# LanceZPF/loongx

Measured on AMD Instinct MI355X. Metric: edited images/s @512x512, 28-step Flux denoise, higher is better.
Workload: dtype bf16

## Files before the change

### include/lx.h

```cpp
#ifndef LX_H_
#define LX_H_
#include <stddef.h>
#include <stdint.h>
#ifdef __cplusplus
extern "C" {
#endif

#define LX_VERSION 404

typedef enum lx_status {
  LX_OK = 0,
  LX_ERR_INVALID = -1,
  LX_ERR_UNSUPPORTED = -2,
  LX_ERR_LAUNCH = -3,
  LX_ERR_NO_DEVICE = -4
} lx_status;

int lx_version(void);
const char* lx_last_error(void);
int lx_device_arch(char* name, size_t n);

enum {
  LX_EPI_STORE_BF16 = 0,
  LX_EPI_STORE_F32 = 1,
  LX_EPI_RESID_F32 = 2,
  LX_EPI_GELU = 0x100,
  LX_W_TILED = 0x200,
  LX_EPI_SPLIT_BF16 = 0x400,
  LX_EPI_STORE_FP8 = 3,
  LX_EPI_QKV = 0x1000,
  LX_OPERANDS_FP8 = 0x800,
  LX_OPERANDS_F16 = 0x2000
};

typedef struct lx_gemm_desc {
  const void* A;
  const void* W;
  const float* bias;
  void* C;
  const float* gate;
  const float* lora_t;
  const float* lora_up;
  int32_t M, N, K;
  int32_t lda, ldw, ldc;
  int32_t rows_per_batch, gate_ld;
  int32_t lora_r, lora_ldt, lora_mod_cols, lora_toff_max;
  int32_t epilogue;
  int32_t gelu_col_start;
  int32_t lora_nsplit;
  int32_t lora_split_stride;
  int32_t k_segs, a_lo_off;
  int32_t c_lo_off;
  float out_scale;
  union {
    const float* col_scale;
    int32_t* f16_ovf;
  };
  const float* qkv_norm_q;
  const float* qkv_norm_k;
  const float* qkv_rope;
  void* qkv_vt;
  void* qkv_k;
  int32_t qkv_d, qkv_vt_ld, qkv_vt_pos0;
  int32_t qkv_k_ld;
  void* qkv_q8;
  void* qkv_k8;
  void* qkv_vt8;
  int32_t qkv_ld8;
  float qkv_q_scale, qkv_k_scale, qkv_v_scale;
} lx_gemm_desc;

#define LX_GEMM_MAX_GROUP 4
int lx_gemm_bf16(const lx_gemm_desc* problems, int n, void* stream);
void lx_gemm_reload_env(void);

size_t lx_gemm_workspace_bytes(void);
int lx_gemm_bf16_ws(const lx_gemm_desc* problems, int n, void* workspace, size_t ws_bytes, void* stream);
int lx_gemm_workspace_status(void* workspace, void* stream);
enum { LX_GEMM_PLAN_NONE = 0, LX_GEMM_PLAN_8WAVE_256 = 1, LX_GEMM_PLAN_8WAVE_128 = 2, LX_GEMM_PLAN_MIXED = 3, LX_GEMM_PLAN_MIXED_2L = 4,
       LX_GEMM_PLAN_G4 = 5, LX_GEMM_PLAN_G4_SPLIT2 = 6, LX_GEMM_PLAN_G4_SPLIT3 = 7 };
int lx_gemm_last_plan(void);

int lx_lora_down(const void* X, int ldx, const void* Adown, float* T, int ldt, int M, int K, int R, int n_split,
                 int split_stride, void* stream);
int lx_lora_down_f16(const void* X, int ldx, const void* Adown, float* T, int ldt, int M, int K, int R, int n_split,
                     int split_stride, void* stream);
int lx_lora_down_terms(const void* const* X, const int* ldx, const void* const* Adown, int n_terms, float* T, int ldt, int M, int K, int R,
                       int slab_stride, void* stream);
typedef struct lx_rowscale_seg { int32_t row0, n_rows, rows_per_batch, _pad; } lx_rowscale_seg;
int lx_lora_scale_rows(float* T, int ldt, int R, int n_slab, int slab_stride, const lx_rowscale_seg* seg, int n_seg,
                       const float* W, int w_ld, int n_batches, int period, void* stream);

int lx_linear_skinny(const float* X, int ldx, const void* W, int ldw, const float* bias, float* Y, int ldy,
                     int M, int N, int K, int act_in, int act_out, int accumulate, void* stream);

int lx_timestep_embed(const float* t, float* out, int B, int dim, void* stream);

int lx_rope_table(const float* ids, int L, int a0, int a1, int a2, double theta, float* cos_t, float* sin_t, void* stream);

int lx_ln_modulate(const float* X, int ldx, const float* shift, const float* scale, int mod_ld, void* Y, int ldy,
                   int M, int D, int rows_per_batch, float eps, void* stream);
typedef struct lx_ln_seg { int32_t row0, n_rows, rows_per_batch, _pad; const float* shift; const float* scale; } lx_ln_seg;
int lx_ln_modulate_segs(const float* X, int ldx, const lx_ln_seg* seg, int n_seg, int mod_ld, void* Y, int ldy, int D,
                        float eps, void* stream);
int lx_ln_modulate_f16_segs(const float* X, int ldx, const lx_ln_seg* seg, int n_seg, int mod_ld, void* Y, int ldy, int D,
                            float eps, int32_t* f16_ovf, void* stream);
int lx_ln_modulate_lora_segs(const float* X, int ldx, const lx_ln_seg* seg, int n_seg, int mod_ld, void* Y, int ldy, int D,
                             float eps, const void* Adown, int R, float* T, int ldt, int lora_row0, int lora_rows, void* stream);
int lx_ln_modulate_lora_f16_segs(const float* X, int ldx, const lx_ln_seg* seg, int n_seg, int mod_ld, void* Y, int ldy, int D,
                                 float eps, const void* Adown, int R, float* T, int ldt, int lora_row0, int lora_rows,
                                 int32_t* f16_ovf, void* stream);
int lx_ln_modulate_delta(const float* X, int ldx, const float* shift, const float* scale, int mod_ld, float* P, int ldp,
                         int M, int D, int rows_per_batch, float eps, float* row_sums , double* sums , void* stream);

int lx_qkv_prep(void* QKV, int ld, int q_col, int k_col, int v_col, int row0, int n_rows, int rows_per_batch,
                int H, const float* wq, const float* wk, float eps, const float* cos_tab, const float* sin_tab,
                void* VT, int vt_ld, int vt_pos0, void* stream);

typedef struct lx_qkv_seg {
  int32_t row0, rows_per_batch, vt_pos0, _pad;
  const float* wq; const float* wk; const float* cos_tab; const float* sin_tab;
} lx_qkv_seg;
int lx_qkv_prep_segs(void* QKV, int ld, int q_col, int k_col, int v_col, const lx_qkv_seg* seg, int n_seg, int n_batches,
                     int H, float eps, void* VT, int vt_ld, void* stream);
int lx_qkv_prep_f16in_segs(void* QKV, int ld, int q_col, int k_col, int v_col, const lx_qkv_seg* seg, int n_seg, int n_batches,
                           int H, float eps, void* VT, int vt_ld, void* stream);

int lx_qkv_prep_kv_segs(void* QKV, int ld, int q_col, int k_col, int v_col, const lx_qkv_seg* seg, int n_seg, int n_batches,
                        int H, float eps, void* K2, int ldk2, int k2_col, void* VT, int vt_ld, void* stream);
int lx_qkv_prep_kv_f16in_segs(void* QKV, int ld, int q_col, int k_col, int v_col, const lx_qkv_seg* seg, int n_seg, int n_batches,
                              int H, float eps, void* K2, int ldk2, int k2_col, void* VT, int vt_ld, void* stream);

typedef struct lx_attn_desc {
  const void* Q; const void* K; const void* VT; void* O;
  int32_t ldq, ldk, ldo, vt_ld;
  int32_t q_col, k_col, o_col;
  int32_t B, H;
  int32_t n_seg;
  int32_t seg_row0[3], seg_len[3], seg_vt0[3];
  float bias[3][3];
  float scale;
  int32_t n_qseg;
  int32_t flags;
  int32_t qseg_mask;
  int32_t* f16_ovf;
} lx_attn_desc;
enum { LX_ATTN_Q_LOG2 = 1, LX_ATTN_BOUNDED = 2, LX_ATTN_INVARIANT = 4, LX_ATTN_O_F16 = 8, LX_ATTN_PREFER_4WAVE = 16, LX_ATTN_P_EXP2 = 32 };
int lx_attn_fwd(const lx_attn_desc* d, void* stream);
enum { LX_ATTN_KERNEL_NONE = 0, LX_ATTN_KERNEL_8WAVE = 1, LX_ATTN_KERNEL_4WAVE = 2 };
int lx_attn_last_kernel(void);

enum { LX_ATTN_MASK_BOOL = 0, LX_ATTN_MASK_F32 = 1, LX_ATTN_MASK_BF16 = 2, LX_ATTN_MASK_F16 = 3 };
typedef struct lx_attn_mask_desc {
  const void* mask;
  int32_t dtype;
  int32_t dims[4];
  int32_t _pad;
  int64_t strides[4];
  void* workspace;
  size_t workspace_bytes;
} lx_attn_mask_desc;
int lx_attn_mask_workspace(const lx_attn_desc* d, const lx_attn_mask_desc* m, size_t* bytes);
int lx_attn_mask_prep(const lx_attn_desc* d, const lx_attn_mask_desc* m, void* stream);
int lx_attn_fwd_masked(const lx_attn_desc* d, const lx_attn_mask_desc* m, void* stream);

int lx_qkv_prep_fp8_segs(const void* QKV, int ld, int q_col, int k_col, int v_col, const lx_qkv_seg* seg, int n_seg,
                         int n_batches, int H, float eps, void* Q8, void* K8, int ld8, void* VT8, int vt8_ld,
                         float q_scale, float k_scale, float v_scale, void* stream);
int lx_qkv_prep_fp8_f16in_segs(const void* QKV, int ld, int q_col, int k_col, int v_col, const lx_qkv_seg* seg, int n_seg,
                               int n_batches, int H, float eps, void* Q8, void* K8, int ld8, void* VT8, int vt8_ld,
                               float q_scale, float k_scale, float v_scale, void* stream);
int lx_attn_fwd_fp8(const lx_attn_desc* d, float qk_descale, float v_descale, void* stream);

int lx_split_bf16(const float* src, int lds, void* dst, int ldd, int lo_off, int M, int K, void* stream);
int lx_ln_modulate_split_segs(const float* X, int ldx, const lx_ln_seg* seg, int n_seg, int mod_ld, void* Y, int ldy, int y_lo_off,
                              int D, float eps, void* stream);
int lx_qkv_prep_f32_segs(float* QKV, int ld, int q_col, int k_col, const lx_qkv_seg* seg, int n_seg, int n_batches, int H, float eps,
                         void* stream);
typedef struct lx_attn_f32_desc {
  const float* QKV; int32_t ld, q_col, k_col, v_col;
  void* O; int32_t ldo, o_col, o_lo_off;
  int32_t B, H, n_seg;
  int32_t seg_row0[3], seg_len[3];
  float bias[3][3];
  float scale;
} lx_attn_f32_desc;
int lx_attn_fwd_f32(const lx_attn_f32_desc* d, void* stream);

int lx_qkv_prep_split_segs(const float* QKV, int ld, int q_col, int k_col, int v_col, const lx_qkv_seg* seg, int n_seg, int n_batches, int H,
                           float eps, void* QK2, int ld2, int q2_col, int k2_col, int lo_off, void* VT2, int vt_ld, long long vt_lo_off,
                           void* stream);
int lx_qkv_prep_split_kv_segs(const float* QKV, int ld, int q_col, int k_col, int v_col, const lx_qkv_seg* seg, int n_seg, int n_batches, int H,
                              float eps, void* Q2, int ldq2, int q2_col, void* K2, int ldk2, int k2_col, int lo_off, void* VT2, int vt_ld,
                              long long vt_lo_off, void* stream);
int lx_attn_fwd_split(const lx_attn_desc* d, int qk_lo_off, long long vt_lo_off, int o_lo_off, void* stream);

int lx_ln_modulate_fp8_segs(const float* X, int ldx, const lx_ln_seg* seg, int n_seg, int mod_ld, void* Y, int ldy, void* Y8, int ldy8,
                            float y8_scale, int D, float eps, void* stream);
int lx_convert_fp8(const void* src, int src_is_bf16, int lds, void* dst, int ldd, float scale, int M, int K, void* stream);
int lx_lora_down_fp8(const void* X8, int ldx, float x_descale, const void* Adown, float* T, int ldt, int M, int K, int R, int n_split,
                     int split_stride, void* stream);

int lx_euler_step(float* x, const void* v, int v_is_bf16, float dsigma, size_t n, void* stream);
int lx_scale_noise(float* out, const float* x0, const float* z, float sigma, size_t n, void* stream);
int lx_euler_step_blend(float* x, const void* v, int v_is_bf16, float dsigma, const float* x0, const float* z, const float* m,
                        float sigma_next, size_t n, void* stream);
int lx_euler_step_cfg(float* x, const void* v, int v_is_bf16, float dsigma, float scale, const float* x0, const float* z, const float* m,
                      float sigma_next, size_t n, void* stream);
int lx_euler_step_cfg3(float* x, const void* v, int v_is_bf16, float dsigma, float scale_brain, float scale_text, const float* x0,
                       const float* z, const float* m, float sigma_next, size_t n, void* stream);
int lx_euler_step_apg(float* x, const void* v, int v_is_bf16, int n_parts, float scale_a, float scale_b, float sigma, float dsigma, float eta,
                      float norm_threshold, float momentum, float* M, double* sums, void* workspace, size_t workspace_bytes, const float* x0,
                      const float* z, const float* m, float sigma_next, int n_images, size_t elems, void* stream);
size_t lx_apg_workspace_bytes(int n_images, size_t elems);
int lx_convert(void* dst, int dst_bf16, const void* src, int src_bf16, size_t n, void* stream);

int lx_s4_scan(const float* u, const double* lam, const double* w, const float* Dskip, float* y,
               int B, int H, int L, int N, void* stream);
int lx_s4_conv(const float* u, const float* Kker, const float* Dskip, float* y, int B, int H, int L, void* stream);
int lx_chanmix(const float* x, const float* W, const float* bias, const float* resid, const float* ln_g,
               const float* ln_b, float* y, int B, int Hin, int Hout, int L, int act, void* stream);
int lx_pyramid_pool(const float* x, float* y, int B, int C, int L, const int* sizes, int n_sizes, int ldy, int y_col0,
                    void* stream);
int lx_layernorm_relu(float* x, const float* g, const float* b, int M, int D, float eps, void* stream);
int lx_linear_f32(const float* X, int ldx, int x_trans, const float* W, int ldw, const float* bias, float* Y, int ldy,
                  int y_trans, int M, int N, int K, int accumulate, void* stream);

int lx_chan_gemm_f32(const float* X, long x_bstride, int ldx, const float* W, int ldw, const float* bias, float* Y, long y_bstride,
                     int ldy, int B, int N, int K, int L, int epilogue, float* part, void* stream);

size_t lx_duan_workspace_bytes(int B, int C, int L, int Hd);
int lx_duan_fwd(const float* x, const float* c, const float* gw1, const float* gb1, const float* gw2, const float* gb2,
                const float* mw1, const float* mb1, const float* mw2, const float* mb2, float* y,
                int B, int C, int L, int Hd, float eps, int keep_k, void* ws, size_t ws_bytes, void* stream);

size_t lx_groupnorm_workspace_bytes(int B, int P, int G);
int lx_groupnorm_silu(const void* x, int x_is_bf16, int B, int P, int C, int G, const float* gamma, const float* beta, float eps,
                      int silu, void* y, void* ws, size_t ws_bytes, void* stream);
int lx_im2col3x3(const void* x, int B, int H, int W, int C, int mode, void* out, int Kpad, void* stream);
int lx_softmax_rows(const float* S, int lds, float scale, void* P, int ldp, int M, int N, void* stream);
int lx_softmax_rows_valid(const float* S, int lds, float scale, void* P, int ldp, int M, int n_valid, int n_store, void* stream);

int lx_groupnorm_silu_split(const float* x, int B, int P, int C, int G, const float* gamma, const float* beta, float eps, int silu,
                            void* y, int ldy, int y_lo_off, void* ws, size_t ws_bytes, void* stream);
int lx_im2col3x3_split(const void* x, int ldx, int x_lo_off, int B, int H, int W, int C, int mode, void* out, int Kpad, void* stream);
int lx_softmax_rows_split(const float* S, int lds, float scale, void* P, int ldp, int p_lo_off, int M, int n_valid, int n_store, void* stream);

int lx_groupnorm_silu_f16(const float* x, int B, int P, int C, int G, const float* gamma, const float* beta, float eps, int silu, void* y,
                          void* ws, size_t ws_bytes, int32_t* f16_ovf, void* stream);
int lx_softmax_rows_f16(const float* S, int lds, float scale, void* P, int ldp, int M, int n_valid, int n_store, void* stream);
int lx_convert_f16(void* dst, const void* src, int src_bf16, size_t n, int32_t* f16_ovf, void* stream);

#ifdef __cplusplus
}
#endif
#endif
```

### loongx_amd/_lib.py

```python
from __future__ import annotations

import ctypes as C
import os

import torch

_HERE = os.path.dirname(os.path.abspath(__file__))
LIB_PATH = os.environ.get("LX_AMD_LIB", os.path.join(_HERE, "lib", "liblx_amd.so"))

LX_EPI_STORE_BF16, LX_EPI_STORE_F32, LX_EPI_RESID_F32, LX_EPI_GELU, LX_W_TILED, LX_EPI_SPLIT_BF16 = 0, 1, 2, 0x100, 0x200, 0x400
LX_EPI_STORE_FP8, LX_OPERANDS_FP8, LX_EPI_QKV, LX_OPERANDS_F16 = 3, 0x800, 0x1000, 0x2000
LX_GEMM_MAX_GROUP = 4
(LX_GEMM_PLAN_NONE, LX_GEMM_PLAN_8WAVE_256, LX_GEMM_PLAN_8WAVE_128, LX_GEMM_PLAN_MIXED, LX_GEMM_PLAN_MIXED_2L, LX_GEMM_PLAN_G4,
 LX_GEMM_PLAN_G4_SPLIT2, LX_GEMM_PLAN_G4_SPLIT3) = range(8)


class GemmDesc(C.Structure):
    _fields_ = [("A", C.c_void_p), ("W", C.c_void_p), ("bias", C.c_void_p), ("C", C.c_void_p),
                ("gate", C.c_void_p), ("lora_t", C.c_void_p), ("lora_up", C.c_void_p),
                ("M", C.c_int32), ("N", C.c_int32), ("K", C.c_int32),
                ("lda", C.c_int32), ("ldw", C.c_int32), ("ldc", C.c_int32),
                ("rows_per_batch", C.c_int32), ("gate_ld", C.c_int32),
                ("lora_r", C.c_int32), ("lora_ldt", C.c_int32), ("lora_mod_cols", C.c_int32),
                ("lora_toff_max", C.c_int32), ("epilogue", C.c_int32), ("gelu_col_start", C.c_int32),
                ("lora_nsplit", C.c_int32), ("lora_split_stride", C.c_int32),
                ("k_segs", C.c_int32), ("a_lo_off", C.c_int32), ("c_lo_off", C.c_int32), ("out_scale", C.c_float),
                ("col_scale", C.c_void_p),
                ("qkv_norm_q", C.c_void_p), ("qkv_norm_k", C.c_void_p), ("qkv_rope", C.c_void_p), ("qkv_vt", C.c_void_p),
                ("qkv_k", C.c_void_p),
                ("qkv_d", C.c_int32), ("qkv_vt_ld", C.c_int32), ("qkv_vt_pos0", C.c_int32), ("qkv_k_ld", C.c_int32),
                ("qkv_q8", C.c_void_p), ("qkv_k8", C.c_void_p), ("qkv_vt8", C.c_void_p),
                ("qkv_ld8", C.c_int32), ("qkv_q_scale", C.c_float), ("qkv_k_scale", C.c_float), ("qkv_v_scale", C.c_float)]


class AttnDesc(C.Structure):
    _fields_ = [("Q", C.c_void_p), ("K", C.c_void_p), ("VT", C.c_void_p), ("O", C.c_void_p),
                ("ldq", C.c_int32), ("ldk", C.c_int32), ("ldo", C.c_int32), ("vt_ld", C.c_int32),
                ("q_col", C.c_int32), ("k_col", C.c_int32), ("o_col", C.c_int32),
                ("B", C.c_int32), ("H", C.c_int32), ("n_seg", C.c_int32),
                ("seg_row0", C.c_int32 * 3), ("seg_len", C.c_int32 * 3), ("seg_vt0", C.c_int32 * 3),
                ("bias", (C.c_float * 3) * 3), ("scale", C.c_float), ("n_qseg", C.c_int32), ("flags", C.c_int32),
                ("qseg_mask", C.c_int32), ("f16_ovf", C.c_void_p)]


LX_ATTN_Q_LOG2, LX_ATTN_BOUNDED, LX_ATTN_INVARIANT, LX_ATTN_O_F16, LX_ATTN_PREFER_4WAVE, LX_ATTN_P_EXP2 = 1, 2, 4, 8, 16, 32
LX_ATTN_MASK_BOOL, LX_ATTN_MASK_F32, LX_ATTN_MASK_BF16, LX_ATTN_MASK_F16 = 0, 1, 2, 3


class AttnMaskDesc(C.Structure):
    _fields_ = [("mask", C.c_void_p), ("dtype", C.c_int32), ("dims", C.c_int32 * 4), ("_pad", C.c_int32),
                ("strides", C.c_int64 * 4), ("workspace", C.c_void_p), ("workspace_bytes", C.c_size_t)]


class AttnF32Desc(C.Structure):
    _fields_ = [("QKV", C.c_void_p), ("ld", C.c_int32), ("q_col", C.c_int32), ("k_col", C.c_int32), ("v_col", C.c_int32),
                ("O", C.c_void_p), ("ldo", C.c_int32), ("o_col", C.c_int32), ("o_lo_off", C.c_int32),
                ("B", C.c_int32), ("H", C.c_int32), ("n_seg", C.c_int32),
                ("seg_row0", C.c_int32 * 3), ("seg_len", C.c_int32 * 3),
                ("bias", (C.c_float * 3) * 3), ("scale", C.c_float)]


class LnSeg(C.Structure):
    _fields_ = [("row0", C.c_int32), ("n_rows", C.c_int32), ("rows_per_batch", C.c_int32), ("_pad", C.c_int32),
                ("shift", C.c_void_p), ("scale", C.c_void_p)]


class RowScaleSeg(C.Structure):
    _fields_ = [("row0", C.c_int32), ("n_rows", C.c_int32), ("rows_per_batch", C.c_int32), ("_pad", C.c_int32)]


class QkvSeg(C.Structure):
    _fields_ = [("row0", C.c_int32), ("rows_per_batch", C.c_int32), ("vt_pos0", C.c_int32), ("_pad", C.c_int32),
                ("wq", C.c_void_p), ("wk", C.c_void_p), ("cos_tab", C.c_void_p), ("sin_tab", C.c_void_p)]


_P, _I, _F, _Z = C.c_void_p, C.c_int, C.c_float, C.c_size_t
_SIGS = {
    "lx_version": (C.c_int, []),
    "lx_last_error": (C.c_char_p, []),
    "lx_device_arch": (C.c_int, [C.c_char_p, _Z]),
    "lx_gemm_bf16": (C.c_int, [C.POINTER(GemmDesc), _I, _P]),
    "lx_gemm_reload_env": (None, []),
    "lx_gemm_workspace_bytes": (_Z, []),
    "lx_gemm_bf16_ws": (C.c_int, [C.POINTER(GemmDesc), _I, _P, _Z, _P]),
    "lx_gemm_workspace_status": (C.c_int, [_P, _P]),
    "lx_gemm_last_plan": (C.c_int, []),
    "lx_lora_down": (C.c_int, [_P, _I, _P, _P, _I, _I, _I, _I, _I, _I, _P]),
    "lx_lora_down_f16": (C.c_int, [_P, _I, _P, _P, _I, _I, _I, _I, _I, _I, _P]),
    "lx_lora_down_terms": (C.c_int, [C.POINTER(C.c_void_p), C.POINTER(C.c_int), C.POINTER(C.c_void_p), _I, _P, _I, _I, _I, _I, _I, _P]),
    "lx_lora_scale_rows": (C.c_int, [_P, _I, _I, _I, _I, C.POINTER(RowScaleSeg), _I, _P, _I, _I, _I, _P]),
    "lx_linear_skinny": (C.c_int, [_P, _I, _P, _I, _P, _P, _I, _I, _I, _I, _I, _I, _I, _P]),
    "lx_timestep_embed": (C.c_int, [_P, _P, _I, _I, _P]),
    "lx_rope_table": (C.c_int, [_P, _I, _I, _I, _I, C.c_double, _P, _P, _P]),
    "lx_ln_modulate": (C.c_int, [_P, _I, _P, _P, _I, _P, _I, _I, _I, _I, _F, _P]),
    "lx_ln_modulate_segs": (C.c_int, [_P, _I, C.POINTER(LnSeg), _I, _I, _P, _I, _I, _F, _P]),
    "lx_ln_modulate_f16_segs": (C.c_int, [_P, _I, C.POINTER(LnSeg), _I, _I, _P, _I, _I, _F, _P, _P]),
    "lx_ln_modulate_lora_segs": (C.c_int, [_P, _I, C.POINTER(LnSeg), _I, _I, _P, _I, _I, _F, _P, _I, _P, _I, _I, _I, _P]),
    "lx_ln_modulate_lora_f16_segs": (C.c_int, [_P, _I, C.POINTER(LnSeg), _I, _I, _P, _I, _I, _F, _P, _I, _P, _I, _I, _I, _P, _P]),
    "lx_ln_modulate_delta": (C.c_int, [_P, _I, _P, _P, _I, _P, _I, _I, _I, _I, _F, _P, _P, _P]),
    "lx_qkv_prep_segs": (C.c_int, [_P, _I, _I, _I, _I, C.POINTER(QkvSeg), _I, _I, _I, _F, _P, _I, _P]),
    "lx_qkv_prep_f16in_segs": (C.c_int, [_P, _I, _I, _I, _I, C.POINTER(QkvSeg), _I, _I, _I, _F, _P, _I, _P]),
    "lx_qkv_prep_kv_segs": (C.c_int, [_P, _I, _I, _I, _I, C.POINTER(QkvSeg), _I, _I, _I, _F, _P, _I, _I, _P, _I, _P]),
    "lx_qkv_prep_kv_f16in_segs": (C.c_int, [_P, _I, _I, _I, _I, C.POINTER(QkvSeg), _I, _I, _I, _F, _P, _I, _I, _P, _I, _P]),
    "lx_qkv_prep": (C.c_int, [_P, _I, _I, _I, _I, _I, _I, _I, _I, _P, _P, _F, _P, _P, _P, _I, _I, _P]),
    "lx_attn_fwd": (C.c_int, [C.POINTER(AttnDesc), _P]),
    "lx_attn_last_kernel": (C.c_int, []),
    "lx_attn_mask_workspace": (C.c_int, [C.POINTER(AttnDesc), C.POINTER(AttnMaskDesc), C.POINTER(C.c_size_t)]),
    "lx_attn_mask_prep": (C.c_int, [C.POINTER(AttnDesc), C.POINTER(AttnMaskDesc), _P]),
    "lx_attn_fwd_masked": (C.c_int, [C.POINTER(AttnDesc), C.POINTER(AttnMaskDesc), _P]),
    "lx_qkv_prep_fp8_segs": (C.c_int, [_P, _I, _I, _I, _I, C.POINTER(QkvSeg), _I, _I, _I, _F, _P, _P, _I, _P, _I, _F, _F, _F, _P]),
    "lx_qkv_prep_fp8_f16in_segs": (C.c_int, [_P, _I, _I, _I, _I, C.POINTER(QkvSeg), _I, _I, _I, _F, _P, _P, _I, _P, _I, _F, _F, _F, _P]),
    "lx_attn_fwd_fp8": (C.c_int, [C.POINTER(AttnDesc), _F, _F, _P]),
    "lx_split_bf16": (C.c_int, [_P, _I, _P, _I, _I, _I, _I, _P]),
    "lx_ln_modulate_split_segs": (C.c_int, [_P, _I, C.POINTER(LnSeg), _I, _I, _P, _I, _I, _I, _F, _P]),
    "lx_qkv_prep_f32_segs": (C.c_int, [_P, _I, _I, _I, C.POINTER(QkvSeg), _I, _I, _I, _F, _P]),
    "lx_attn_fwd_f32": (C.c_int, [C.POINTER(AttnF32Desc), _P]),
    "lx_qkv_prep_split_segs": (C.c_int, [_P, _I, _I, _I, _I, C.POINTER(QkvSeg), _I, _I, _I, _F, _P, _I, _I, _I, _I, _P, _I, C.c_longlong, _P]),
    "lx_qkv_prep_split_kv_segs": (C.c_int, [_P, _I, _I, _I, _I, C.POINTER(QkvSeg), _I, _I, _I, _F, _P, _I, _I, _P, _I, _I, _I, _P, _I, C.c_longlong, _P]),
    "lx_attn_fwd_split": (C.c_int, [C.POINTER(AttnDesc), _I, C.c_longlong, _I, _P]),
    "lx_groupnorm_workspace_bytes": (_Z, [_I, _I, _I]),
    "lx_groupnorm_silu": (C.c_int, [_P, _I, _I, _I, _I, _I, _P, _P, _F, _I, _P, _P, _Z, _P]),
    "lx_im2col3x3": (C.c_int, [_P, _I, _I, _I, _I, _I, _P, _I, _P]),
    "lx_softmax_rows": (C.c_int, [_P, _I, _F, _P, _I, _I, _I, _P]),
    "lx_softmax_rows_valid": (C.c_int, [_P, _I, _F, _P, _I, _I, _I, _I, _P]),
    "lx_groupnorm_silu_split": (C.c_int, [_P, _I, _I, _I, _I, _P, _P, _F, _I, _P, _I, _I, _P, _Z, _P]),
    "lx_im2col3x3_split": (C.c_int, [_P, _I, _I, _I, _I, _I, _I, _I, _P, _I, _P]),
    "lx_softmax_rows_split": (C.c_int, [_P, _I, _F, _P, _I, _I, _I, _I, _I, _P]),
    "lx_groupnorm_silu_f16": (C.c_int, [_P, _I, _I, _I, _I, _P, _P, _F, _I, _P, _P, _Z, _P, _P]),
    "lx_softmax_rows_f16": (C.c_int, [_P, _I, _F, _P, _I, _I, _I, _I, _P]),
    "lx_convert_f16": (C.c_int, [_P, _P, _I, _Z, _P, _P]),
    "lx_ln_modulate_fp8_segs": (C.c_int, [_P, _I, C.POINTER(LnSeg), _I, _I, _P, _I, _P, _I, _F, _I, _F, _P]),
    "lx_convert_fp8": (C.c_int, [_P, _I, _I, _P, _I, _F, _I, _I, _P]),
    "lx_lora_down_fp8": (C.c_int, [_P, _I, _F, _P, _P, _I, _I, _I, _I, _I, _I, _P]),
    "lx_euler_step": (C.c_int, [_P, _P, _I, _F, _Z, _P]),
    "lx_scale_noise": (C.c_int, [_P, _P, _P, _F, _Z, _P]),
    "lx_euler_step_blend": (C.c_int, [_P, _P, _I, _F, _P, _P, _P, _F, _Z, _P]),
    "lx_euler_step_cfg": (C.c_int, [_P, _P, _I, _F, _F, _P, _P, _P, _F, _Z, _P]),
    "lx_euler_step_cfg3": (C.c_int, [_P, _P, _I, _F, _F, _F, _P, _P, _P, _F, _Z, _P]),
    "lx_apg_workspace_bytes": (_Z, [_I, _Z]),
    "lx_euler_step_apg": (C.c_int, [_P, _P, _I, _I] + [_F] * 7 + [_P, _P, _P, _Z, _P, _P, _P, _F, _I, _Z, _P]),
    "lx_convert": (C.c_int, [_P, _I, _P, _I, _Z, _P]),
    "lx_s4_scan": (C.c_int, [_P, _P, _P, _P, _P, _I, _I, _I, _I, _P]),
    "lx_s4_conv": (C.c_int, [_P, _P, _P, _P, _I, _I, _I, _P]),
    "lx_chanmix": (C.c_int, [_P, _P, _P, _P, _P, _P, _P, _I, _I, _I, _I, _I, _P]),
    "lx_pyramid_pool": (C.c_int, [_P, _P, _I, _I, _I, C.POINTER(C.c_int), _I, _I, _I, _P]),
    "lx_layernorm_relu": (C.c_int, [_P, _P, _P, _I, _I, _F, _P]),
    "lx_linear_f32": (C.c_int, [_P, _I, _I, _P, _I, _P, _P, _I, _I, _I, _I, _I, _I, _P]),
    "lx_chan_gemm_f32": (C.c_int, [_P, C.c_long, _I, _P, _I, _P, _P, C.c_long, _I, _I, _I, _I, _I, _I, _P, _P]),
    "lx_duan_workspace_bytes": (_Z, [_I, _I, _I, _I]),
    "lx_duan_fwd": (C.c_int, [_P] * 11 + [_I, _I, _I, _I, _F, _I, _P, _Z, _P]),
}

EXPORTS = tuple(_SIGS)


class LxError(RuntimeError):
    pass


def _load():
    if not os.path.exists(LIB_PATH):
        raise ImportError(f"liblx_amd.so not found at {LIB_PATH}: build it with `python -c 'import __graft_entry__ as g; "
                          f"g.build()'` or loongx_amd/csrc/build.sh -- there is no CPU/torch fallback for the hot path")
    lib = C.CDLL(LIB_PATH)
    for name, (res, args) in _SIGS.items():
        fn = getattr(lib, name)
        fn.restype, fn.argtypes = res, args
    return lib


lib = _load()


def check(status: int, what: str = "") -> None:
    if status != 0:
        raise LxError(f"{what or 'lx call'} failed ({status}): {lib.lx_last_error().decode()}")
```

### loongx_amd/csrc/gemm.hip

```cpp
#include "gemm8.h"


static double round_us(int bm, int K) { return bm == 256 ? 15.0 + 1.81 * (K / 64) : 10.5 + 1.06 * (K / 64); }

struct GemmEnv { int bm, g4, sk, g4_fault; };
static int env_int(const char* name, int dflt) {
  const char* s = getenv(name);
  return s ? atoi(s) : dflt;
}
static GemmEnv read_gemm_env() { return GemmEnv{env_int("LX_GEMM_BM", 0), env_int("LX_GEMM4", 1), env_int("LX_GEMM4_SK", 1), env_int("LX_GEMM4_FAULT", 0)}; }
static GemmEnv g_gemm_env = read_gemm_env();
static const GemmEnv& gemm_env() { return g_gemm_env; }
extern "C" void lx_gemm_reload_env(void) { g_gemm_env = read_gemm_env(); }

namespace {
constexpr size_t SK_FLAGS_OFF = (size_t)256 * SK_SLOT_FLOATS * sizeof(float);
constexpr size_t SK_WS_BYTES = SK_FLAGS_OFF + (256 + 64) * sizeof(int);
static_assert(SK_WS_BYTES % 256 == 0, "workspace size keeps the 256-byte alignment contract");
constexpr int SK_MIN_KT_ALL = 96;
constexpr int SK_MAX_ROUNDS = 16;

int device_cus() {
  static int n = -1;
  if (n < 0) {
    int dev = 0;
    hipDeviceProp_t pr;
    n = (hipGetDevice(&dev) == hipSuccess && hipGetDeviceProperties(&pr, dev) == hipSuccess) ? pr.multiProcessorCount : 0;
  }
  return n;
}
}

static long tiles_of(const lx_gemm_desc& p, int bm) { return (long)((p.M + bm - 1) / bm) * ((p.N + BN - 1) / BN); }

static lx_gemm_desc sub_rows(const lx_gemm_desc& p, int r0, int rows) {
  lx_gemm_desc q = p;
  q.A = (const uint16_t*)p.A + (size_t)r0 * p.lda;
  const int epi = p.epilogue & 0xff;
  q.C = epi == LX_EPI_STORE_BF16 ? (void*)((uint16_t*)p.C + (size_t)r0 * p.ldc) : (void*)((float*)p.C + (size_t)r0 * p.ldc);
  if (p.lora_t) q.lora_t = p.lora_t + (size_t)r0 * p.lora_ldt;
  if (p.qkv_k) q.qkv_k = (uint16_t*)p.qkv_k + (size_t)r0 * p.qkv_k_ld;
  if (p.qkv_q8) {
    q.qkv_q8 = (uint8_t*)p.qkv_q8 + (size_t)r0 * p.qkv_ld8;
    q.qkv_k8 = (uint8_t*)p.qkv_k8 + (size_t)r0 * p.qkv_ld8;
  }
  q.M = rows;
  return q;
}

static int launch_plan(const GemmArgs& a, int bm, hipStream_t s, int variant = LX_GV_BF16) {
  if (a.n == 0) return LX_OK;
  if (variant == LX_GV_SPLIT) lx_gemm8_launch_split(bm, a, s);
  else if (variant == LX_GV_F16) lx_gemm8_launch_f16(bm, a, s);
  else if (variant == LX_GV_FP8) lx_gemm8_launch_fp8(bm, a, s);
  else lx_gemm8_launch_bf16(bm, a, s);
  LX_LAUNCH_CHECK("lx_gemm_bf16");
  return LX_OK;
}

void lx_gemm8_launch_bf16(int bm, const GemmArgs& a, hipStream_t s) {
  const int t = a.tile_start[a.n];
  if (bm == 256) hipLaunchKernelGGL((lx_gemm_kernel<256, false>), dim3(t), dim3(NTHREADS), 0, s, a);
  else hipLaunchKernelGGL((lx_gemm_kernel<128, false>), dim3(t), dim3(NTHREADS), 0, s, a);
}
void lx_gemm8_mixed_launch_bf16(const GemmArgs& big, const GemmArgs& tail, int n_big_pad, hipStream_t s) {
  hipLaunchKernelGGL(lx_gemm_mixed_kernel<false>, dim3(n_big_pad + tail.tile_start[tail.n]), dim3(NTHREADS), 0, s, big, tail, n_big_pad);
}

static void plan_add(GemmArgs& a, const lx_gemm_desc& p, int m_base, int bm) {
  a.p[a.n] = p;
  a.m_base[a.n] = m_base;
  a.tile_start[a.n + 1] = a.tile_start[a.n] + (int)tiles_of(p, bm);
  ++a.n;
  for (int i = a.n + 1; i <= MAX_SUB; ++i) a.tile_start[i] = a.tile_start[a.n];
}

static thread_local int lx_gemm_last = LX_GEMM_PLAN_NONE;
extern "C" int lx_gemm_last_plan(void) { return lx_gemm_last; }
static int planned(int rc, int plan) {
  if (rc == LX_OK) lx_gemm_last = plan;
  return rc;
}

extern "C" size_t lx_gemm_workspace_bytes(void) { return SK_WS_BYTES; }

extern "C" int lx_gemm_workspace_status(void* workspace, void* stream) {
  LX_CHECK_ARG(workspace, "lx_gemm_workspace_status: NULL workspace");
  int* err = (int*)((char*)workspace + SK_FLAGS_OFF) + 256;
  int v = 0;
  hipStream_t s = (hipStream_t)stream;
  if (hipMemcpyAsync(&v, err, sizeof(int), hipMemcpyDeviceToHost, s) != hipSuccess || hipStreamSynchronize(s) != hipSuccess) {
    lx_set_error("lx_gemm_workspace_status: reading the error word failed: %s", hipGetErrorString(hipGetLastError()));
    return LX_ERR_LAUNCH;
  }
  if (v == 0) return LX_OK;
  (void)hipMemsetAsync((char*)workspace + SK_FLAGS_OFF, 0, (256 + 64) * sizeof(int), s);
  (void)hipStreamSynchronize(s);
  lx_set_error("lx_gemm_bf16_ws: a split-K pair workgroup timed out waiting for its partner (CUs held by other work?); the results "
               "of that launch are invalid. Re-run with the workspace omitted (lx_gemm_bf16) or LX_GEMM4_SK=0");
  return LX_ERR_LAUNCH;
}

extern "C" int lx_gemm_bf16(const lx_gemm_desc* problems, int n, void* stream) { return lx_gemm_bf16_ws(problems, n, nullptr, 0, stream); }

extern "C" int lx_gemm_bf16_ws(const lx_gemm_desc* problems, int n, void* workspace, size_t ws_bytes, void* stream) {
  LX_CHECK_ARG(problems && n >= 1 && n <= LX_GEMM_MAX_GROUP, "lx_gemm_bf16: n=%d out of range [1,%d]", n, LX_GEMM_MAX_GROUP);
  long t256 = 0, t128 = 0;
  int kmax = 0;
  bool split = false, fp8 = false, f16 = false, qkv = false;
  for (int i = 0; i < n; ++i) fp8 = fp8 || (problems[i].epilogue & LX_OPERANDS_FP8) != 0;
  for (int i = 0; i < n; ++i) f16 = f16 || (problems[i].epilogue & LX_OPERANDS_F16) != 0;
  for (int i = 0; i < n; ++i) {
    const lx_gemm_desc& p = problems[i];
    if (f16) {
      LX_CHECK_ARG((p.epilogue & LX_OPERANDS_F16) != 0 && !(p.epilogue & LX_OPERANDS_FP8) && p.k_segs <= 1 && !(p.epilogue & LX_EPI_SPLIT_BF16),
                   "lx_gemm_bf16[%d]: LX_OPERANDS_F16 must be set on every problem of a launch and excludes the e4m3 and split-bf16 modes", i);
      if (p.f16_ovf) LX_CHECK_ARG(((uintptr_t)p.f16_ovf & 3) == 0, "lx_gemm_bf16[%d]: f16_ovf must be 4-byte aligned", i);
    }
    if (fp8) {
      LX_CHECK_ARG((p.epilogue & LX_OPERANDS_FP8) != 0 && p.k_segs <= 1 && !(p.epilogue & LX_EPI_SPLIT_BF16), "lx_gemm_bf16[%d]: LX_OPERANDS_FP8 must be set on every problem of a launch and excludes the split-bf16 mode", i);
      LX_CHECK_ARG(p.K % 128 == 0 && p.lda % 16 == 0 && p.ldw % 16 == 0, "lx_gemm_bf16[%d]: fp8 operands need K %% 128 == 0 and lda / ldw %% 16 == 0 (K=%d)", i, p.K);
      if (p.col_scale) LX_CHECK_ARG(((uintptr_t)p.col_scale & 15) == 0, "lx_gemm_bf16[%d]: col_scale must be 16-byte aligned", i);
      if (p.lora_t) LX_CHECK_ARG(p.lora_r <= 4 && p.lora_nsplit <= 4, "lx_gemm_bf16[%d]: the fp8 path applies LoRA in the tile prologue only (rank <= 4, <= 4 slabs)", i);
      if ((p.epilogue & 0xff) == LX_EPI_STORE_FP8) LX_CHECK_ARG(p.out_scale > 0.f && p.ldc % 8 == 0, "lx_gemm_bf16[%d]: LX_EPI_STORE_FP8 needs out_scale > 0 and ldc %% 8 == 0", i);
    }
    LX_CHECK_ARG(p.k_segs >= 0 && p.k_segs <= 3, "lx_gemm_bf16[%d]: k_segs=%d must be 0..3", i, p.k_segs);
    const int segs = p.k_segs > 1 ? p.k_segs : 1;
    if (segs > 1 || (p.epilogue & LX_EPI_SPLIT_BF16)) split = true;
    if (segs > 1) LX_CHECK_ARG(p.a_lo_off >= p.K && p.a_lo_off % 8 == 0 && p.lda >= p.a_lo_off + p.K, "lx_gemm_bf16[%d]: a_lo_off=%d needs K <= a_lo_off, a_lo_off + K <= lda, multiple of 8", i, p.a_lo_off);
    if (segs == 3) LX_CHECK_ARG(p.ldw >= 2 * p.K, "lx_gemm_bf16[%d]: k_segs = 3 reads W as [N, 2K] = [W_hi | W_lo]: ldw=%d < 2K", i, p.ldw);
    if (p.epilogue & LX_EPI_SPLIT_BF16) LX_CHECK_ARG((p.epilogue & 0xff) == LX_EPI_STORE_BF16 && p.c_lo_off >= p.N && p.c_lo_off % 8 == 0 && p.ldc >= p.c_lo_off + p.N,
                                                     "lx_gemm_bf16[%d]: LX_EPI_SPLIT_BF16 needs a bf16 store and N <= c_lo_off, c_lo_off + N <= ldc, multiple of 8", i);
    LX_CHECK_ARG(p.A && p.W && p.C, "lx_gemm_bf16[%d]: NULL operand", i);
    LX_CHECK_ARG(p.M > 0 && p.N > 0 && p.K > 0, "lx_gemm_bf16[%d]: bad shape M=%d N=%d K=%d", i, p.M, p.N, p.K);
    LX_CHECK_ARG(p.K % BK == 0, "lx_gemm_bf16[%d]: K=%d must be a multiple of %d", i, p.K, BK);
    LX_CHECK_ARG(p.N % 8 == 0, "lx_gemm_bf16[%d]: N=%d must be a multiple of 8", i, p.N);
    LX_CHECK_ARG(p.lda % 8 == 0 && p.ldw % 8 == 0 && p.lda >= p.K && p.ldw >= p.K, "lx_gemm_bf16[%d]: lda/ldw must be >= K and multiples of 8", i);
    LX_CHECK_ARG(((uintptr_t)p.A & 15) == 0 && ((uintptr_t)p.W & 15) == 0 && ((uintptr_t)p.C & 15) == 0, "lx_gemm_bf16[%d]: operands must be 16-byte aligned", i);
    LX_CHECK_ARG(p.ldc % 8 == 0 && p.ldc >= p.N, "lx_gemm_bf16[%d]: ldc=%d must be >= N and a multiple of 8", i, p.ldc);
    const int epi = p.epilogue & 0xff;
    LX_CHECK_ARG(epi >= LX_EPI_STORE_BF16 && (epi <= LX_EPI_RESID_F32 || (fp8 && epi == LX_EPI_STORE_FP8)), "lx_gemm_bf16[%d]: unknown epilogue %d", i, p.epilogue);
    LX_CHECK_ARG(p.rows_per_batch > 0, "lx_gemm_bf16[%d]: rows_per_batch must be > 0", i);
    if (p.epilogue & LX_W_TILED) LX_CHECK_ARG(p.N % BN == 0 && p.ldw == (segs == 3 ? 2 * p.K : p.K), "lx_gemm_bf16[%d]: LX_W_TILED needs N %% 256 == 0 and ldw == K (2K with k_segs = 3)", i);
    if (p.gate) LX_CHECK_ARG(p.gate_ld >= p.N && p.gate_ld % 4 == 0, "lx_gemm_bf16[%d]: gate_ld=%d", i, p.gate_ld);
    if (p.lora_t) {
      LX_CHECK_ARG(p.lora_up && p.lora_r >= 1 && p.lora_r <= 64, "lx_gemm_bf16[%d]: LoRA needs lora_up and 1 <= r <= 64", i);
      LX_CHECK_ARG(p.lora_r <= 16 || !(segs > 1 || (p.epilogue & LX_EPI_SPLIT_BF16)), "lx_gemm_bf16[%d]: the split-bf16 mode applies LoRA of rank <= 16 (r=%d)", i, p.lora_r);
      LX_CHECK_ARG(p.lora_mod_cols <= 0 || p.lora_mod_cols % BN == 0, "lx_gemm_bf16[%d]: lora_mod_cols must be a multiple of %d", i, BN);
    }
    if (p.epilogue & LX_EPI_QKV) {
      LX_CHECK_ARG(!fp8 && segs == 1 && !(p.epilogue & LX_EPI_SPLIT_BF16) && epi == LX_EPI_STORE_BF16, "lx_gemm_bf16[%d]: LX_EPI_QKV goes with plain bf16 operands and LX_EPI_STORE_BF16", i);
      LX_CHECK_ARG(p.qkv_d > 0 && p.qkv_d % BN == 0 && (p.N >= 3 * p.qkv_d || p.N % BN == 0), "lx_gemm_bf16[%d]: LX_EPI_QKV needs qkv_d %% 256 == 0 and whole projection tiles (qkv_d=%d N=%d)", i, p.qkv_d, p.N);
      LX_CHECK_ARG(p.rows_per_batch % 32 == 0 && p.M % 32 == 0, "lx_gemm_bf16[%d]: LX_EPI_QKV needs rows_per_batch %% 32 == 0 and M %% 32 == 0 (%d, %d)", i, p.rows_per_batch, p.M);
      const bool q8 = p.qkv_q8 != nullptr;
      LX_CHECK_ARG(p.qkv_norm_q && p.qkv_norm_k && (p.qkv_vt || q8) && p.qkv_rope && ((uintptr_t)p.qkv_norm_q & 15) == 0 && ((uintptr_t)p.qkv_norm_k & 15) == 0 && ((uintptr_t)p.qkv_vt & 15) == 0 &&
                   ((uintptr_t)p.qkv_rope & 15) == 0, "lx_gemm_bf16[%d]: LX_EPI_QKV needs 16-byte aligned qkv_norm_q / qkv_norm_k / qkv_rope / qkv_vt", i);
      if (q8) {
        LX_CHECK_ARG(p.qkv_k8 && p.qkv_vt8 && (((uintptr_t)p.qkv_q8 | (uintptr_t)p.qkv_k8 | (uintptr_t)p.qkv_vt8) & 15) == 0 && p.qkv_ld8 % 16 == 0 && p.qkv_ld8 >= p.qkv_d,
                     "lx_gemm_bf16[%d]: LX_EPI_QKV e4m3 outputs need 16-byte aligned qkv_q8 / qkv_k8 / qkv_vt8 and qkv_ld8 %% 16 == 0, >= qkv_d", i);
        LX_CHECK_ARG(p.qkv_q_scale > 0.f && p.qkv_k_scale > 0.f && p.qkv_v_scale > 0.f && !p.qkv_k, "lx_gemm_bf16[%d]: LX_EPI_QKV e4m3 outputs need positive scales and no separate bf16 key image", i);
      }
      LX_CHECK_ARG(p.qkv_vt_ld > 0 && p.qkv_vt_ld % 64 == 0 && p.qkv_vt_pos0 >= 0 && p.qkv_vt_pos0 % 64 == 0 && p.qkv_vt_pos0 + p.rows_per_batch <= p.qkv_vt_ld,
                   "lx_gemm_bf16[%d]: qkv_vt_ld / qkv_vt_pos0 must be multiples of 64 with the stream inside a V^T row", i);
      if (p.qkv_k) LX_CHECK_ARG(((uintptr_t)p.qkv_k & 15) == 0 && p.qkv_k_ld % 8 == 0 && p.qkv_k_ld >= p.qkv_d, "lx_gemm_bf16[%d]: qkv_k must be 16-byte aligned with qkv_k_ld %% 8 == 0, >= qkv_d", i);
      qkv = true;
    }
    if (p.bias) LX_CHECK_ARG(((uintptr_t)p.bias & 15) == 0, "lx_gemm_bf16[%d]: bias must be 16-byte aligned", i);
    t256 += tiles_of(p, 256);
    t128 += tiles_of(p, 128);
    kmax = p.K * segs > kmax ? p.K * segs : kmax;
  }
  hipStream_t s = (hipStream_t)stream;
  if (fp8) {
    const int ncu = device_cus() > 0 ? device_cus() : 256;
    const double ca = (double)((t256 + ncu - 1) / ncu) * round_us(256, kmax / 4), cb = (double)((t128 + ncu - 1) / ncu) * round_us(128, kmax / 4);
    const int bm = gemm_env().bm ? gemm_env().bm : (cb < ca ? 128 : 256);
    GemmArgs all;
    all.n = 0;
    all.tile_start[0] = 0;
    for (int i = 1; i <= MAX_SUB; ++i) all.tile_start[i] = 0;
    for (int i = 0; i < n; ++i) plan_add(all, problems[i], 0, bm);
    return planned(launch_plan(all, bm, s, LX_GV_FP8), bm == 256 ? LX_GEMM_PLAN_8WAVE_256 : LX_GEMM_PLAN_8WAVE_128);
  }
  const int NCU = device_cus() > 0 ? device_cus() : 256;
  const GemmEnv& env = gemm_env();
  const int forced = env.bm;
  if (env.g4 && forced == 0 && (workspace || env.g4 == 2)) {
    bool ok = true;
    for (int i = 0; i < n; ++i) {
      const lx_gemm_desc& p = problems[i];
      ok = ok && (p.epilogue & 0xff) <= LX_EPI_RESID_F32 && p.K / BK >= 2 && !((p.epilogue & LX_EPI_QKV) && p.qkv_q8);
      if (p.lora_t)
        ok = ok && p.lora_r <= 8 && p.lora_r % 2 == 0 && p.lora_nsplit >= 1 && p.lora_nsplit <= 4 && p.lora_ldt % 2 == 0 && p.lora_split_stride % 2 == 0 &&
             ((((uintptr_t)p.lora_t) | ((uintptr_t)p.lora_up)) & 7) == 0;
    }
    const long rounds = (t256 + NCU - 1) / NCU;
    bool fills = env.g4 == 2 || (t256 >= NCU && (rounds * NCU - t256 <= NCU / 4 || rounds >= 8));
    bool uniform_k4 = true;
    for (int i = 1; i < n; ++i) uniform_k4 = uniform_k4 && problems[i].K == problems[0].K;
    const long tail = t256 % NCU, full = t256 - tail;
    for (int i = 1; i < n; ++i) uniform_k4 = uniform_k4 && problems[i].k_segs == problems[0].k_segs;
    const int kt_all = kmax / BK;
    const bool can_split = env.sk && workspace && ws_bytes >= SK_WS_BYTES && ((uintptr_t)workspace & 255) == 0 && uniform_k4 && kt_all >= 16 &&
                           tail > 0 && tail * 2 <= 256 && tail * 2 <= NCU && rounds <= SK_MAX_ROUNDS;
    bool split_all = can_split && full == 0 && kt_all >= SK_MIN_KT_ALL;
    const int tail_div = !qkv && kt_all >= 96 ? 2 : 3;
    bool split_tail = can_split && full > 0 && tail * tail_div <= NCU;
    int np = 2;
    if (!split && env.sk != 2 && kt_all >= 24 && tail * 3 <= 256 && tail * 3 <= NCU && (split_all || split_tail) && (kt_all >= 96 || tail * 6 <= NCU)) np = 3;
    if (split) {
      const double r4 = 8.9 + 1.31 * kt_all;
      const bool sk_tail = can_split && tail > 0;
      const double c4 = (double)(full / NCU) * r4 + (tail == 0 ? 0.0 : sk_tail ? 8.9 + 1.31 * (kt_all - kt_all / 2) + 6.0 : r4);
      const double c8a = (double)((t256 + NCU - 1) / NCU) * (5.8 + 1.55 * kt_all), c8b = (double)((t128 + NCU - 1) / NCU) * (10.5 + 1.06 * kt_all);
      fills = env.g4 == 2 || c4 < (c8a < c8b ? c8a : c8b);
      split_all = fills && sk_tail && full == 0;
      split_tail = fills && sk_tail && full > 0;
      if (!fills) split_all = split_tail = false;
    }
    if (ok && (fills || split_all || split_tail)) {
      GemmArgs all;
      all.n = 0;
      all.tile_start[0] = 0;
      for (int i = 1; i <= MAX_SUB; ++i) all.tile_start[i] = 0;
      for (int i = 0; i < n; ++i) plan_add(all, problems[i], 0, 256);
      float* slots = nullptr;
      int *flags = nullptr, *err = nullptr;
      unsigned grid = (unsigned)t256;
      int sk_full = (int)t256, sk_parts = 1;
      if (split_all || split_tail) {
        slots = (float*)workspace;
        flags = (int*)((char*)workspace + SK_FLAGS_OFF);
        err = flags + 256;
        grid = (unsigned)(full + np * tail);
        sk_full = (int)full;
        sk_parts = env.g4_fault ? 3 : 2;
      }
      if (split) lx_gemm4_launch_split(all, grid, sk_full, sk_parts, slots, flags, err, s);
      else if (f16) lx_gemm4_launch_f16(all, grid, sk_full, sk_parts, slots, flags, err, s, np);
      else lx_gemm4_launch_bf16(all, grid, sk_full, sk_parts, slots, flags, err, s, np);
      LX_LAUNCH_CHECK("lx_gemm_bf16");
      return planned(LX_OK, !(split_all || split_tail) ? LX_GEMM_PLAN_G4 : np == 3 ? LX_GEMM_PLAN_G4_SPLIT3 : LX_GEMM_PLAN_G4_SPLIT2);
    }
  }
  if (split) {
    const double ca = (double)((t256 + NCU - 1) / NCU) * round_us(256, kmax), cb = (double)((t128 + NCU - 1) / NCU) * round_us(128, kmax);
    const int bm = forced ? forced : (cb < ca ? 128 : 256);
    GemmArgs all;
    all.n = 0;
    all.tile_start[0] = 0;
    for (int i = 1; i <= MAX_SUB; ++i) all.tile_start[i] = 0;
    for (int i = 0; i < n; ++i) plan_add(all, problems[i], 0, bm);
    return planned(launch_plan(all, bm, s, LX_GV_SPLIT), bm == 256 ? LX_GEMM_PLAN_8WAVE_256 : LX_GEMM_PLAN_8WAVE_128);
  }
  if (workspace) LX_CHECK_ARG(ws_bytes >= SK_WS_BYTES && ((uintptr_t)workspace & 255) == 0, "lx_gemm_bf16_ws: workspace needs %zu bytes (lx_gemm_workspace_bytes()), 256-byte aligned", SK_WS_BYTES);
  const int variant = f16 ? LX_GV_F16 : LX_GV_BF16;
  const double c_a = (double)((t256 + NCU - 1) / NCU) * round_us(256, kmax);
  const double c_b = (double)((t128 + NCU - 1) / NCU) * round_us(128, kmax);
  GemmArgs big, tail;
  big.n = tail.n = 0;
  big.tile_start[0] = tail.tile_start[0] = 0;
  for (int i = 1; i <= MAX_SUB; ++i) big.tile_start[i] = tail.tile_start[i] = 0;
  double c_c = 1e30;
  const long full = (t256 / NCU) * NCU;
  if (forced == 0 && full > 0 && t256 > full) {
    long remain = t256;
    int keep_rows[LX_GEMM_MAX_GROUP];
    for (int i = 0; i < n; ++i) keep_rows[i] = problems[i].M;
    for (int i = n - 1; i >= 0 && remain > full; --i) {
      const int tn = (problems[i].N + BN - 1) / BN;
      while (remain > full && keep_rows[i] > 0) {
        const int last_rows = keep_rows[i] % 256 ? keep_rows[i] % 256 : 256;
        keep_rows[i] -= last_rows;
        remain -= tn;
      }
    }
    long tail_tiles = 0;
    for (int i = 0; i < n; ++i) {
      if (keep_rows[i] > 0) plan_add(big, sub_rows(problems[i], 0, keep_rows[i]), 0, 256);
      if (keep_rows[i] < problems[i].M) {
        const lx_gemm_desc q = sub_rows(problems[i], keep_rows[i], problems[i].M - keep_rows[i]);
        plan_add(tail, q, keep_rows[i], 128);
        tail_tiles += tiles_of(q, 128);
      }
    }
    c_c = (double)((remain + NCU - 1) / NCU) * round_us(256, kmax) + (double)((tail_tiles + NCU - 1) / NCU) * round_us(128, kmax) + 2.0;
  }
  int choice = forced == 256 ? 0 : forced == 128 ? 1 : (c_c < c_a && c_c < c_b) ? 2 : (c_b < c_a ? 1 : 0);
  if (choice == 2) {
    if (big.n > 0 && tail.n > 0) {
      const int n_big = big.tile_start[big.n], n_big_pad = (n_big + 7) & ~7;
      if (f16) lx_gemm8_mixed_launch_f16(big, tail, n_big_pad, s);
      else lx_gemm8_mixed_launch_bf16(big, tail, n_big_pad, s);
      LX_LAUNCH_CHECK("lx_gemm_bf16");
      return planned(LX_OK, LX_GEMM_PLAN_MIXED);
    }
    const int rc = launch_plan(big, 256, s, variant);
    if (rc != LX_OK) return rc;
    return planned(launch_plan(tail, 128, s, variant), LX_GEMM_PLAN_MIXED_2L);
  }
  GemmArgs all;
  all.n = 0;
  all.tile_start[0] = 0;
  for (int i = 1; i <= MAX_SUB; ++i) all.tile_start[i] = 0;
  for (int i = 0; i < n; ++i) plan_add(all, problems[i], 0, choice == 0 ? 256 : 128);
  return planned(launch_plan(all, choice == 0 ? 256 : 128, s, variant), choice == 0 ? LX_GEMM_PLAN_8WAVE_256 : LX_GEMM_PLAN_8WAVE_128);
}
```

### loongx_amd/csrc/gemm4.h

```cpp
#pragma once
#include "gemm_common.h"

namespace {

constexpr int G4_STAGE = 256 * BK * 2 + BN * BK * 2;
constexpr int G4_LDS = 2 * G4_STAGE;
constexpr int G4_PLD = 132;
constexpr int G4_PATCHES = 4 * 2 * 16 * G4_PLD * 4;
constexpr int G4_SLOT = 8 * 1024;
constexpr int G4_SMEM = G4_PATCHES + 4 * 2 * G4_SLOT > G4_LDS ? G4_PATCHES + 4 * 2 * G4_SLOT : G4_LDS;
static_assert(G4_LDS <= G4_SMEM && G4_SMEM <= 160 * 1024 && G4_PATCHES % 1024 == 0 && G4_PATCHES + 4 * 2 * G4_SLOT <= G4_SMEM,
              "LDS budget / epilogue patches / row ring");

#ifdef LX_G4_PROBE
__device__ unsigned long long lx_g4_probe_buf[8192 * 8];
#define G4_STAMP(k) if (threadIdx.x == 0 && blockIdx.x < 8192) { asm volatile("s_waitcnt lgkmcnt(0)" ::: "memory"); lx_g4_probe_buf[blockIdx.x * 8 + (k)] = __builtin_amdgcn_s_memtime(); }
#else
#define G4_STAMP(k)
#endif


template <bool SPLIT, bool F16 = false, int NP = 2>
__global__ __launch_bounds__(G4_THREADS) void lx_gemm4_kernel(const GemmArgs args, const int sk_full, const int sk_parts, float* __restrict__ sk_slots,
                                                              int* __restrict__ sk_flags, int* __restrict__ sk_err) {
#if defined(__HIP_DEVICE_COMPILE__)
  __shared__ __attribute__((aligned(1024))) char smem[G4_SMEM];
  constexpr int BM = 256, A_BYTES = BM * BK * 2;
  const int pid = blockIdx.x;
  G4_STAMP(0)
  const int total = args.tile_start[MAX_SUB];
  int lid, part = 0;
  if (pid < sk_full) {
    const int q = sk_full >> 3, r = sk_full & 7;
    const int xcd = pid & 7, inx = pid >> 3;
    lid = (xcd < r ? xcd * (q + 1) : r * (q + 1) + (xcd - r) * q) + inx;
  } else {
    const int r = pid - sk_full;
    lid = sk_full + r / NP;
    part = r % NP;
  }
  (void)total;
  const bool split_tile = pid >= sk_full && sk_parts >= 2;
  const int g = tile_group(args, lid);
  lx_gemm_desc P = args.p[g];
  int tm, tn;
  tile_coords<BM>(P, lid - args.tile_start[g], tm, tn);
  const int tid = threadIdx.x, lane = tid & 63;
  const int wave = __builtin_amdgcn_readfirstlane(tid >> 6);
  const int wm = wave >> 1, wn = wave & 1, l15 = lane & 15, lq = lane >> 4;
  int m0 = tm * BM, n0 = tn * BN;
  int M = P.M, N = P.N;
  const int K = P.K;
  const bool w_tiled = (P.epilogue & LX_W_TILED) != 0;
  const int nk1 = K / BK;
  const int nkt = SPLIT ? nk1 * max(P.k_segs, 1) : nk1;
  const int kt_begin = !split_tile ? 0 : NP == 2 ? (part ? nkt >> 1 : 0) : (part * nkt) / NP;
  const int kt_end = !split_tile ? nkt : NP == 2 ? (part ? nkt : nkt >> 1) : ((part + 1) * nkt) / NP;

  uint32_t aoff[8], woff[8];
  {
    const int rsub = lane >> 3, pslot = lane & 7;
#pragma unroll
    for (int j = 0; j < 8; ++j) {
      const int row = (j * 4 + wave) * 8 + rsub;
      const int lslot = pslot ^ ((row >> 1) & 7);
      aoff[j] = (uint32_t)((min(m0 + row, M - 1) - m0) * P.lda + lslot * 8) * 2u;
      woff[j] = w_tiled ? (uint32_t)((j * 4 + wave) * 512 + lane * 8) * 2u : (uint32_t)((min(n0 + row, N - 1) - n0) * P.ldw + lslot * 8) * 2u;
    }
  }
  const __bf16* a_org = (const __bf16*)P.A + (size_t)m0 * P.lda;
  const int kw_tiles = SPLIT && P.k_segs == 3 ? 2 * nk1 : nk1;
  const __bf16* w_org = w_tiled ? (const __bf16*)P.W + ((size_t)tn * kw_tiles) * (BN * BK) : (const __bf16*)P.W + (size_t)n0 * P.ldw;
  const lx_rsrc_t rs_a = lx_make_rsrc(a_org), rs_w = lx_make_rsrc(w_org);
  const int w_kstride_b = (w_tiled ? BN * BK : BK) * 2;
  const int a_lo_b = SPLIT ? P.a_lo_off * 2 : 0;
  auto a_soff = [&](int t) -> int {
    if constexpr (!SPLIT) return t * (BK * 2);
    else {
      const int seg = t >= 2 * nk1 ? 2 : (t >= nk1 ? 1 : 0);
      return (t - seg * nk1) * (BK * 2) + (seg == 1 ? a_lo_b : 0);
    }
  };
  auto w_soff = [&](int t) -> int {
    if constexpr (!SPLIT) return t * w_kstride_b;
    else {
      const int seg = t >= 2 * nk1 ? 2 : (t >= nk1 ? 1 : 0);
      return (t - seg * nk1 + (seg == 2 ? nk1 : 0)) * w_kstride_b;
    }
  };
  auto piece = [&](int p_, int a_so, int w_so, int stage) {
    if (p_ < 8) lx_buf_to_lds(rs_a, (lptr_t)(smem + stage * G4_STAGE + (p_ * 4 + wave) * 1024), aoff[p_], a_so);
    else lx_buf_to_lds(rs_w, (lptr_t)(smem + stage * G4_STAGE + A_BYTES + ((p_ - 8) * 4 + wave) * 1024), woff[p_ - 8], w_so);
  };
  int a_ad[2], w_ad[2];
  {
    const int ar = wm * 128 + l15, wr = wn * 128 + l15;
#pragma unroll
    for (int ks = 0; ks < 2; ++ks) {
      a_ad[ks] = ar * 128 + (((ks * 4 + lq) ^ ((ar >> 1) & 7)) * 16);
      w_ad[ks] = A_BYTES + wr * 128 + (((ks * 4 + lq) ^ ((wr >> 1) & 7)) * 16);
    }
  }
  f32x4 acc[8][8];
#pragma unroll
  for (int i = 0; i < 8; ++i)
#pragma unroll
    for (int j = 0; j < 8; ++j) acc[i][j] = f32x4{0.f, 0.f, 0.f, 0.f};
  bf16x8 af[2][8], wf[2][8];
  auto rd = [&](int stage, int ks, int idx) {
    const char* base = smem + stage * G4_STAGE;
    if (idx < 8) wf[ks][idx] = *(const bf16x8*)(base + w_ad[ks] + idx * 2048);
    else af[ks][idx - 8] = *(const bf16x8*)(base + a_ad[ks] + (idx - 8) * 2048);
  };
  auto mm = [&](int ks, int n_) {
    const int j = n_ >> 3, i = n_ & 7;
    if constexpr (F16) asm volatile("v_mfma_f32_16x16x32_f16 %0, %1, %2, %0" : "+a"(acc[i][j]) : "v"(wf[ks][j]), "v"(af[ks][i]));
    else asm volatile("v_mfma_f32_16x16x32_bf16 %0, %1, %2, %0" : "+a"(acc[i][j]) : "v"(wf[ks][j]), "v"(af[ks][i]));
  };
#define G4_SB() __builtin_amdgcn_sched_barrier(0)
  const bool has_lora = P.lora_t != nullptr && kt_begin == 0;
  u32x2 lu[8], lt[8][4];
  if (has_lora) {
    const int R = P.lora_r, nsplit = P.lora_nsplit;
    const int toff = R * min(n0 / max(P.lora_mod_cols, 1), P.lora_toff_max);
    const int rk = min(2 * lq, R - 2);
#pragma unroll
    for (int j = 0; j < 8; ++j) lu[j] = *(const u32x2*)(P.lora_up + (size_t)min(n0 + wn * 128 + j * 16 + l15, N - 1) * R + rk);
#pragma unroll
    for (int i = 0; i < 8; ++i) {
      const float* tp = P.lora_t + (size_t)min(m0 + wm * 128 + i * 16 + l15, M - 1) * P.lora_ldt + toff + rk;
#pragma unroll
      for (int q = 0; q < 4; ++q) lt[i][q] = *(const u32x2*)(tp + (size_t)min(q, nsplit - 1) * P.lora_split_stride);
    }
  }
  {
    const int t1 = min(kt_begin + 1, kt_end - 1);
    const int a0 = a_soff(kt_begin), w0 = w_soff(kt_begin), a1 = a_soff(t1), w1 = w_soff(t1);
#pragma unroll
    for (int p_ = 0; p_ < 16; ++p_) piece(p_, a0, w0, 0);
#pragma unroll
    for (int p_ = 0; p_ < 16; ++p_) piece(p_, a1, w1, 1);
  }
  asm volatile("s_waitcnt vmcnt(16)" ::: "memory");
  __builtin_amdgcn_s_barrier();
  G4_SB();
  G4_STAMP(1)
#pragma unroll
  for (int x = 0; x < 16; ++x) rd(0, 0, x);
  if (has_lora) {
    const int R = P.lora_r, nsplit = P.lora_nsplit;
    const bool live = 2 * lq < R;
    auto frag_u = [&](u32x2 v) {
      const float a = live ? __uint_as_float(v[0]) : 0.f, b = live ? __uint_as_float(v[1]) : 0.f;
      const uint16_t ah = f32_to_bf16(a), bh = f32_to_bf16(b);
      const uint16_t al = f32_to_bf16(a - bf16_to_f32(ah)), bl = f32_to_bf16(b - bf16_to_f32(bh));
      const u32x4 w = {(uint32_t)ah * 0x10001u, (uint32_t)al * 0x10001u, (uint32_t)bh * 0x10001u, (uint32_t)bl * 0x10001u};
      return __builtin_bit_cast(bf16x8, w);
    };
    auto frag_t = [&](float a, float b) {
      a = live ? a : 0.f; b = live ? b : 0.f;
      const uint16_t ah = f32_to_bf16(a), bh = f32_to_bf16(b);
      const uint32_t pa = (uint32_t)ah | ((uint32_t)f32_to_bf16(a - bf16_to_f32(ah)) << 16);
      const uint32_t pb = (uint32_t)bh | ((uint32_t)f32_to_bf16(b - bf16_to_f32(bh)) << 16);
      const u32x4 w = {pa, pa, pb, pb};
      return __builtin_bit_cast(bf16x8, w);
    };
    bf16x8 uf[8], tf[8];
#pragma unroll
    for (int j = 0; j < 8; ++j) uf[j] = frag_u(lu[j]);
#pragma unroll
    for (int i = 0; i < 8; ++i) {
      float a = __uint_as_float(lt[i][0][0]), b = __uint_as_float(lt[i][0][1]);
#pragma unroll
      for (int q = 1; q < 4; ++q)
        if (q < nsplit) { a += __uint_as_float(lt[i][q][0]); b += __uint_as_float(lt[i][q][1]); }
      tf[i] = frag_t(a, b);
    }
#pragma unroll
    for (int j = 0; j < 8; ++j)
#pragma unroll
      for (int i = 0; i < 8; ++i) acc[i][j] = __builtin_amdgcn_mfma_f32_16x16x32_bf16(uf[j], tf[i], acc[i][j], 0, 0, 0);
    asm volatile("s_nop 15\n s_nop 7" ::: "memory");
  }
  asm volatile("s_waitcnt lgkmcnt(0)" ::: "memory");
  G4_STAMP(2)
  int c = 0;
  for (int kt = kt_begin; kt < kt_end; ++kt) {
    const int n = c ^ 1;
    const int kt2 = min(kt + 2, kt_end - 1);
    const int a_so2 = a_soff(kt2), w_so2 = w_soff(kt2);
#pragma unroll
    for (int m = 0; m < 64; ++m) {
      if (m == 16) {
        G4_SB();
        asm volatile("s_waitcnt lgkmcnt(0)" ::: "memory");
        __builtin_amdgcn_s_barrier();
        G4_SB();
      }
      mm(0, m); G4_SB();
      if (m < 16) { rd(c, 1, m); G4_SB(); }
      if (m >= 16 && (m - 16) % 6 == 0) { piece((m - 16) / 6, a_so2, w_so2, c); G4_SB(); }
    }
#pragma unroll
    for (int m = 0; m < 64; ++m) {
      if (m == 43) {
        G4_SB();
        asm volatile("s_waitcnt vmcnt(16)" ::: "memory");
        __builtin_amdgcn_s_barrier();
        G4_SB();
      }
      mm(1, m); G4_SB();
      if (m < 40 && m % 5 == 0) { piece(8 + m / 5, a_so2, w_so2, c); G4_SB(); }
      if (m >= 43 && m < 59) { rd(n, 0, m - 43); G4_SB(); }
    }
    asm volatile("s_waitcnt lgkmcnt(0)" ::: "memory");
    c = n;
  }
#undef G4_SB
  G4_STAMP(3)
  asm volatile("s_nop 15\n s_nop 7\n s_waitcnt vmcnt(0)" ::: "memory");
  __syncthreads();
  G4_STAMP(4)

  const float* partner = nullptr;
  const float* partner2 = nullptr;
  float* my_slot = nullptr;
  if (split_tile) {
    my_slot = sk_slots + (size_t)(pid - sk_full) * SK_SLOT_FLOATS;
    if constexpr (NP == 2) {
      partner = sk_slots + (size_t)((pid - sk_full) ^ 1) * SK_SLOT_FLOATS;
    } else {
      const int gb = (pid - sk_full) - part;
      partner = sk_slots + (size_t)(gb + (part + 1) % NP) * SK_SLOT_FLOATS;
      partner2 = sk_slots + (size_t)(gb + (part + 2) % NP) * SK_SLOT_FLOATS;
    }
  }
  auto pld4 = [&](size_t off_floats, const float* from) {
    const u32x4 v = __builtin_amdgcn_raw_buffer_load_b128(lx_make_rsrc(from), (int)(off_floats * 4), 0, PAIR_AUX_SC1);
    return f32x4{__uint_as_float(v[0]), __uint_as_float(v[1]), __uint_as_float(v[2]), __uint_as_float(v[3])};
  };
  const int lm0 = wm * 128, ln0 = wn * 128;
  auto exchange = [&]() {
    asm volatile("s_waitcnt vmcnt(0)" ::: "memory");
    __syncthreads();
    __builtin_amdgcn_fence(__ATOMIC_RELEASE, "workgroup");
    if (tid == 0) {
      const int me = pid - sk_full, other = NP == 2 ? (me ^ 1) : (me - part + (part + 1) % NP), other2 = me - part + (part + 2) % NP;
      bool ok = __hip_atomic_load(sk_err, __ATOMIC_RELAXED, __HIP_MEMORY_SCOPE_AGENT) == 0;
      if (ok) {
        if (!(sk_parts == 3 && part == 1))
          __hip_atomic_store(sk_flags + me, NP - 1, __ATOMIC_RELAXED, __HIP_MEMORY_SCOPE_AGENT);
        int spins = 0;
        while (__hip_atomic_load(sk_flags + other, __ATOMIC_RELAXED, __HIP_MEMORY_SCOPE_AGENT) == 0) {
          __builtin_amdgcn_s_sleep(1);
          if (++spins > (1 << 20)) { ok = false; break; }
        }
        if constexpr (NP == 3) {
          while (ok && __hip_atomic_load(sk_flags + other2, __ATOMIC_RELAXED, __HIP_MEMORY_SCOPE_AGENT) == 0) {
            __builtin_amdgcn_s_sleep(1);
            if (++spins > (1 << 20)) { ok = false; break; }
          }
        }
        if (ok) {
          if constexpr (NP == 2) __hip_atomic_store(sk_flags + other, 0, __ATOMIC_RELAXED, __HIP_MEMORY_SCOPE_AGENT);
          else {
            __hip_atomic_fetch_add(sk_flags + other, -1, __ATOMIC_RELAXED, __HIP_MEMORY_SCOPE_AGENT);
            __hip_atomic_fetch_add(sk_flags + other2, -1, __ATOMIC_RELAXED, __HIP_MEMORY_SCOPE_AGENT);
          }
        } else __hip_atomic_store(sk_err, 1, __ATOMIC_RELAXED, __HIP_MEMORY_SCOPE_AGENT);
      }
    }
    __syncthreads();
    G4_STAMP(6)
    __builtin_amdgcn_fence(__ATOMIC_ACQUIRE, "workgroup");
  };

  const int epi = P.epilogue & 0xff;
  const bool do_gelu = (P.epilogue & LX_EPI_GELU) != 0;
  const int mw0 = m0 + wm * 128, nw0 = n0 + wn * 128;
  float* patch = (float*)smem + wave * (2 * 16 * G4_PLD);
  const bool bf16_out = epi == LX_EPI_STORE_BF16;
  const int c8 = (lane & 15) * 8, c4 = (lane & 31) * 4;
  const int ncol = nw0 + (bf16_out ? c8 : c4);
  const bool col_ok = ncol < N;
  f32x4 bias0 = {0.f, 0.f, 0.f, 0.f}, bias1 = {0.f, 0.f, 0.f, 0.f};
  if (P.bias && col_ok) {
    bias0 = *(const f32x4*)(P.bias + ncol);
    if (bf16_out) bias1 = *(const f32x4*)(P.bias + ncol + 4);
  }
  asm volatile("s_waitcnt vmcnt(0)" : "+v"(bias0), "+v"(bias1)::"memory");
  const bool gelu0 = do_gelu && ncol >= P.gelu_col_start;
  const int m_base = args.m_base[g];
  static_assert(!(F16 && SPLIT), "fp16 operands exclude the split-bf16 mode");
  float f16_mx = 0.f;
  const bool qkv_tile = (P.epilogue & LX_EPI_QKV) != 0 && n0 < 3 * P.qkv_d;
  const int qkind = qkv_tile ? n0 / P.qkv_d : -1;
  f32x4 nw0v = {1.f, 1.f, 1.f, 1.f}, nw1v = {1.f, 1.f, 1.f, 1.f};
  if (qkv_tile && qkind != 1) {
    const float* nwp = (qkind == 2 ? P.qkv_norm_q : P.qkv_norm_k) + c8;
    nw0v = *(const f32x4*)nwp; nw1v = *(const f32x4*)(nwp + 4);
    asm volatile("s_waitcnt vmcnt(0)" : "+v"(nw0v), "+v"(nw1v)::"memory");
  }
#ifdef LX_G4_RESID_GLOBAL
  constexpr bool RING_RES = false;
#else
  constexpr bool RING_RES = true;
#endif
#ifdef LX_G4_ROPE_GLOBAL
  constexpr bool RING_ROPE = false;
#else
  constexpr bool RING_ROPE = true;
#endif
  char* const ring = smem + G4_PATCHES + wave * (2 * G4_SLOT);
  const bool ring_res = RING_RES && epi == LX_EPI_RESID_F32 && !qkv_tile;
  const bool ring_rope = RING_ROPE && qkv_tile && qkind != 1;
  const int ring_lane = ring_rope ? ((lane >> 4) * 128 + c8) * 4 : min(ncol, max(N - 4, 0)) * 4;
  const int ring_mlast = M - 1 - mw0;
  auto ring_issue = [&](int b, int s) {
    const lx_rsrc_t rs_row = lx_make_rsrc(ring_rope ? (const void*)P.qkv_rope : (const void*)((const float*)P.C + (size_t)min(mw0, M - 1) * P.ldc));
    if (ring_rope) {
      const int gm = m_base + mw0 + b * 16, p0 = gm - (gm / P.rows_per_batch) * P.rows_per_batch;
#pragma unroll
      for (int p_ = 0; p_ < 8; ++p_)
        lx_buf_to_lds(rs_row, (lptr_t)(ring + s * G4_SLOT + p_ * 1024), (uint32_t)ring_lane, (p0 + (p_ >> 1) * 4) * 512 + (p_ & 1) * 16);
    } else {
#pragma unroll
      for (int t = 0; t < 8; ++t) {
        const int r = min(b * 16 + t * 2 + (lane >> 5), ring_mlast);
        lx_buf_to_lds(rs_row, (lptr_t)(ring + s * G4_SLOT + t * 1024), (uint32_t)(r * P.ldc * 4 + ring_lane), 0);
      }
    }
  };
  auto ring_wait = [&](auto ko_, bool nxt, bool stores, auto st_) {
    constexpr int ko = decltype(ko_)::value, ST = decltype(st_)::value, S = ST * (ko < 2 ? ko : 2);
    if (stores) {
      if (nxt) asm volatile("s_waitcnt vmcnt(%0)" ::"n"(S + 8) : "memory");
      else asm volatile("s_waitcnt vmcnt(%0)" ::"n"(S) : "memory");
    } else {
      if (nxt) asm volatile("s_waitcnt vmcnt(8)" ::: "memory");
      else asm volatile("s_waitcnt vmcnt(0)" ::: "memory");
    }
  };
  const bool gate_tile = RING_RES && epi == LX_EPI_RESID_F32 && !qkv_tile && P.gate != nullptr &&
                         (m_base + m0) / P.rows_per_batch == (m_base + m0 + BM - 1) / P.rows_per_batch;
  f32x4 gate_t = {0.f, 0.f, 0.f, 0.f};
  if (gate_tile && col_ok) gate_t = *(const f32x4*)(P.gate + (size_t)((m_base + m0) / P.rows_per_batch) * P.gate_ld + ncol);
  asm volatile("s_waitcnt vmcnt(0)" : "+v"(gate_t)::"memory");
  auto put = [&](auto ic_) {
    constexpr int i = decltype(ic_)::value;
    float* pt = patch + (i & 1) * (16 * G4_PLD);
    asm volatile("" : "+a"(acc[i][0]), "+a"(acc[i][1]), "+a"(acc[i][2]), "+a"(acc[i][3]), "+a"(acc[i][4]), "+a"(acc[i][5]), "+a"(acc[i][6]), "+a"(acc[i][7]));
#pragma unroll
    for (int j = 0; j < 8; ++j) *(f32x4*)(pt + l15 * G4_PLD + j * 16 + 4 * lq) = acc[i][j];
  };
  auto park = [&](auto ic_, auto nx_) {
    constexpr int i = decltype(ic_)::value, nx = decltype(nx_)::value;
    const float* pt = patch + (i & 1) * (16 * G4_PLD);
    __builtin_amdgcn_wave_barrier();
    if constexpr (nx >= 0) { if (mw0 + nx * 16 < M) put(std::integral_constant<int, nx>{}); }
    __builtin_amdgcn_sched_barrier(0);
    if (mw0 + i * 16 >= M) return;
    const lx_rsrc_t rs_slot = lx_make_rsrc(my_slot);
#pragma unroll
    for (int t = 0; t < 8; ++t) {
      const int row = t * 2 + (lane >> 5);
      const f32x4 v = *(const f32x4*)(pt + row * G4_PLD + c4);
      __builtin_amdgcn_raw_buffer_store_b128(u32x4{__float_as_uint(v[0]), __float_as_uint(v[1]), __float_as_uint(v[2]), __float_as_uint(v[3])}, rs_slot,
                                             (int)(((size_t)(wm * 128 + i * 16 + row) * 256 + wn * 128 + c4) * 4), 0, PAIR_AUX_SC1);
    }
  };
  auto block = [&](auto ic_, auto nx_, auto ko_, auto n2_) {
    constexpr int i = decltype(ic_)::value, nx = decltype(nx_)::value, ko = decltype(ko_)::value, n2 = decltype(n2_)::value;
    const int mb = mw0 + i * 16;
    if (mb >= M) return;
    const float* pt = patch + (i & 1) * (16 * G4_PLD);
    const char* const slot = ring + (ko & 1) * G4_SLOT + lane * 16;
    const bool ring_nxt = nx >= 0 && mw0 + nx * 16 < M;
    f32x4 res[8], gat[8];
    if (epi == LX_EPI_RESID_F32 && !qkv_tile) {
      const int rpb = P.rows_per_batch;
#pragma unroll
      for (int t = 0; t < 8; ++t) {
        const int m = mb + t * 2 + (lane >> 5);
        if (m < M && col_ok) {
          if (!RING_RES) {
            res[t] = *(const f32x4*)((const float*)P.C + (size_t)m * P.ldc + ncol);
            if (P.gate) gat[t] = *(const f32x4*)(P.gate + (size_t)((m_base + m) / rpb) * P.gate_ld + ncol);
          }
        }
      }
    }
    __builtin_amdgcn_wave_barrier();
    if constexpr (nx >= 0) { if (mw0 + nx * 16 < M) put(std::integral_constant<int, nx>{}); }
    __builtin_amdgcn_sched_barrier(0);
    if (partner) {
      f32x4 pa[4][2], pb[4][2];
#pragma unroll
      for (int t = 0; t < 4; ++t) {
        const size_t po = (size_t)(lm0 + i * 16 + t * 4 + (lane >> 4)) * 256 + ln0 + c8;
        pa[t][0] = pld4(po, partner); pa[t][1] = pld4(po + 4, partner);
        if constexpr (NP == 3) { pb[t][0] = pld4(po, partner2); pb[t][1] = pld4(po + 4, partner2); }
      }
      float* pw = patch + (i & 1) * (16 * G4_PLD);
#pragma unroll
      for (int t = 0; t < 4; ++t) {
        float* q_ = pw + (t * 4 + (lane >> 4)) * G4_PLD + c8;
        f32x4 v0 = *(const f32x4*)q_, v1 = *(const f32x4*)(q_ + 4);
#pragma unroll
        for (int c_ = 0; c_ < 4; ++c_) { v0[c_] += pa[t][0][c_]; v1[c_] += pa[t][1][c_]; }
        if constexpr (NP == 3) {
#pragma unroll
          for (int c_ = 0; c_ < 4; ++c_) { v0[c_] += pb[t][0][c_]; v1[c_] += pb[t][1][c_]; }
        }
        *(f32x4*)q_ = v0; *(f32x4*)(q_ + 4) = v1;
      }
      __builtin_amdgcn_wave_barrier();
    }
    if (qkv_tile) {
      const int D = P.qkv_d, L = P.rows_per_batch, H = D >> 7;
      const int gm = m_base + mb, b = gm / L, p0 = gm - b * L;
      const int h = (nw0 - qkind * D) >> 7;
      if (qkind == 1) {
        const int gk = lane & 1;
        float e[4][8];
#pragma unroll
        for (int t = 0; t < 4; ++t)
#pragma unroll
          for (int k = 0; k < 8; ++k) {
            const int rk = lx_vt_interleave(gk * 8 + k), dk = t * 32 + (lane >> 1);
            e[t][k] = pt[rk * G4_PLD + dk];
          }
#pragma unroll
        for (int t = 0; t < 4; ++t) {
          const int d = t * 32 + (lane >> 1);
          const float bd = P.bias ? P.bias[nw0 + d] : 0.f;
          u32x4 o = {pack_bf16x2(e[t][0] + bd, e[t][1] + bd), pack_bf16x2(e[t][2] + bd, e[t][3] + bd), pack_bf16x2(e[t][4] + bd, e[t][5] + bd),
                     pack_bf16x2(e[t][6] + bd, e[t][7] + bd)};
          *(u32x4*)((uint16_t*)P.qkv_vt + ((size_t)(b * H + h) * 128 + d) * P.qkv_vt_ld + P.qkv_vt_pos0 + p0 + gk * 8) = o;
        }
      } else {
        uint16_t* const out = (qkind == 0 && P.qkv_k) ? (uint16_t*)P.qkv_k : (uint16_t*)P.C;
        const int out_ld = (qkind == 0 && P.qkv_k) ? P.qkv_k_ld : P.ldc;
        f32x4 cs[4][2], pv[4][2];
        if constexpr (RING_ROPE) {
          ring_wait(ko_, ring_nxt, true, std::integral_constant<int, 4>{});
#pragma unroll
          for (int t = 0; t < 4; ++t) { cs[t][0] = *(const f32x4*)(slot + (t * 2) * 1024); cs[t][1] = *(const f32x4*)(slot + (t * 2 + 1) * 1024); }
        } else {
#pragma unroll
          for (int t = 0; t < 4; ++t) {
            const float* rp = P.qkv_rope + (size_t)(p0 + t * 4 + (lane >> 4)) * 128 + c8;
            cs[t][0] = *(const f32x4*)rp; cs[t][1] = *(const f32x4*)(rp + 4);
          }
        }
#pragma unroll
        for (int t = 0; t < 4; ++t) {
          const int row = t * 4 + (lane >> 4);
          pv[t][0] = *(const f32x4*)(pt + row * G4_PLD + c8); pv[t][1] = *(const f32x4*)(pt + row * G4_PLD + c8 + 4);
        }
        if constexpr (RING_ROPE && n2 >= 0) {
          if (mw0 + n2 * 16 < M) {
            asm volatile("s_waitcnt lgkmcnt(0)" : "+v"(cs[0][0]), "+v"(cs[0][1]), "+v"(cs[1][0]), "+v"(cs[1][1]), "+v"(cs[2][0]), "+v"(cs[2][1]), "+v"(cs[3][0]), "+v"(cs[3][1])::"memory");
            ring_issue(n2, ko & 1);
          }
        }
        float yy[4][8];
#pragma unroll
        for (int t = 0; t < 4; ++t) {
          f32x4 v0 = pv[t][0], v1 = pv[t][1];
          float ss = 0.f;
#pragma unroll
          for (int c_ = 0; c_ < 4; ++c_) { v0[c_] += bias0[c_]; v1[c_] += bias1[c_]; ss = __builtin_fmaf(v0[c_], v0[c_], ss); ss = __builtin_fmaf(v1[c_], v1[c_], ss); }
#ifdef LX_G4_ROW16_SHFL
          ss += __shfl_xor(ss, 1, 64); ss += __shfl_xor(ss, 2, 64); ss += __shfl_xor(ss, 4, 64); ss += __shfl_xor(ss, 8, 64);
#else
          ss = row16_sum(ss);
#endif
          const float r = rsqrtf(ss * (1.0f / 128.0f) + 1e-6f);
          float x[8];
          float (&y)[8] = yy[t];
#pragma unroll
          for (int c_ = 0; c_ < 4; ++c_) { x[c_] = v0[c_] * r * nw0v[c_]; x[4 + c_] = v1[c_] * r * nw1v[c_]; }
#pragma unroll
          for (int q = 0; q < 4; ++q) {
            const float co = q < 2 ? cs[t][0][2 * q] : cs[t][1][2 * q - 4], si = q < 2 ? cs[t][0][2 * q + 1] : cs[t][1][2 * q - 3];
            y[2 * q] = x[2 * q] * co - x[2 * q + 1] * si;
            y[2 * q + 1] = x[2 * q + 1] * co + x[2 * q] * si;
          }
        }
#pragma unroll
        for (int t = 0; t < 4; ++t) {
          const int m = mb + t * 4 + (lane >> 4);
          const float (&y)[8] = yy[t];
          u32x4 o = {pack_bf16x2(y[0], y[1]), pack_bf16x2(y[2], y[3]), pack_bf16x2(y[4], y[5]), pack_bf16x2(y[6], y[7])};
          if (m < M) *(u32x4*)(out + (size_t)m * out_ld + ncol) = o;
        }
      }
      return;
    }
    if (bf16_out) {
      f32x4 pv[4][2];
#pragma unroll
      for (int t = 0; t < 4; ++t) {
        const int row = t * 4 + (lane >> 4);
        pv[t][0] = *(const f32x4*)(pt + row * G4_PLD + c8); pv[t][1] = *(const f32x4*)(pt + row * G4_PLD + c8 + 4);
      }
#pragma unroll
      for (int t = 0; t < 4; ++t) {
        const int row = t * 4 + (lane >> 4), m = mb + row;
        f32x4 v0 = pv[t][0], v1 = pv[t][1];
        if (m < M && col_ok) {
#pragma unroll
          for (int c_ = 0; c_ < 4; ++c_) { v0[c_] += bias0[c_]; v1[c_] += bias1[c_]; }
          if (gelu0) { v0 = gelu_tanh4(v0); v1 = gelu_tanh4(v1); }
          u32x4 o = {pack_op16x2<F16>(v0[0], v0[1], f16_mx), pack_op16x2<F16>(v0[2], v0[3], f16_mx), pack_op16x2<F16>(v1[0], v1[1], f16_mx),
                     pack_op16x2<F16>(v1[2], v1[3], f16_mx)};
          *(u32x4*)((uint16_t*)P.C + (size_t)m * P.ldc + ncol) = o;
          if constexpr (SPLIT) {
            if (P.epilogue & LX_EPI_SPLIT_BF16) {
              float r[8];
#pragma unroll
              for (int c_ = 0; c_ < 4; ++c_) {
                r[c_] = v0[c_] - bf16_to_f32(f32_to_bf16(v0[c_]));
                r[4 + c_] = v1[c_] - bf16_to_f32(f32_to_bf16(v1[c_]));
              }
              u32x4 ol = {pack_bf16x2(r[0], r[1]), pack_bf16x2(r[2], r[3]), pack_bf16x2(r[4], r[5]), pack_bf16x2(r[6], r[7])};
              *(u32x4*)((uint16_t*)P.C + (size_t)m * P.ldc + ncol + P.c_lo_off) = ol;
            }
          }
        }
      }
    } else {
      f32x4 pv[8];
#pragma unroll
      for (int t = 0; t < 8; ++t) pv[t] = *(const f32x4*)(pt + (t * 2 + (lane >> 5)) * G4_PLD + c4);
      if (epi == LX_EPI_RESID_F32) {
        if constexpr (RING_RES) {
          if (P.gate && !gate_tile) {
            const int rpb = P.rows_per_batch;
#pragma unroll
            for (int t = 0; t < 8; ++t) {
              const int m = mb + t * 2 + (lane >> 5);
              if (m < M && col_ok) gat[t] = *(const f32x4*)(P.gate + (size_t)((m_base + m) / rpb) * P.gate_ld + ncol);
            }
            asm volatile("s_waitcnt vmcnt(0)" ::: "memory");
#pragma unroll
            for (int t = 0; t < 8; ++t) asm volatile("" : "+v"(gat[t]));
          } else ring_wait(ko_, ring_nxt, nw0 < N, std::integral_constant<int, 8>{});
#pragma unroll
          for (int t = 0; t < 8; ++t) res[t] = *(const f32x4*)(slot + t * 1024);
          asm volatile("s_waitcnt lgkmcnt(0)" : "+v"(res[0]), "+v"(res[1]), "+v"(res[2]), "+v"(res[3]), "+v"(res[4]), "+v"(res[5]), "+v"(res[6]), "+v"(res[7])::"memory");
          if constexpr (n2 >= 0) { if (mw0 + n2 * 16 < M) ring_issue(n2, ko & 1); }
        } else {
          asm volatile("s_waitcnt vmcnt(0)" ::: "memory");
#pragma unroll
          for (int t = 0; t < 8; ++t) asm volatile("" : "+v"(res[t]), "+v"(gat[t]));
        }
      }
#pragma unroll
      for (int t = 0; t < 8; ++t) {
        const int row = t * 2 + (lane >> 5), m = mb + row;
        f32x4 v = pv[t];
        if (m < M && col_ok) {
#pragma unroll
          for (int c_ = 0; c_ < 4; ++c_) v[c_] += bias0[c_];
          if (gelu0) v = gelu_tanh4(v);
          if (epi == LX_EPI_RESID_F32) {
            f32x4 o = res[t];
            if (P.gate) {
              const f32x4 gv = gate_tile ? gate_t : gat[t];
#pragma unroll
              for (int c_ = 0; c_ < 4; ++c_) o[c_] = __builtin_fmaf(gv[c_], v[c_], o[c_]);
            } else {
#pragma unroll
              for (int c_ = 0; c_ < 4; ++c_) o[c_] += v[c_];
            }
            v = o;
          }
          *(f32x4*)((float*)P.C + (size_t)m * P.ldc + ncol) = v;
        }
      }
    }
  };
#define G4_B(I, NX, KO, N2) block(std::integral_constant<int, I>{}, std::integral_constant<int, NX>{}, std::integral_constant<int, KO>{}, std::integral_constant<int, N2>{})
#define G4_K(I, NX) park(std::integral_constant<int, I>{}, std::integral_constant<int, NX>{})
#define G4_R(B0, B1) if (ring_res || ring_rope) { if (mw0 + (B0) * 16 < M) ring_issue(B0, 0); if (mw0 + (B1) * 16 < M) ring_issue(B1, 1); }
  if (!split_tile) {
    G4_R(0, 1)
    if (mw0 < M) put(std::integral_constant<int, 0>{});
    G4_B(0, 1, 0, 2); G4_B(1, 2, 1, 3); G4_B(2, 3, 2, 4); G4_B(3, 4, 3, 5); G4_B(4, 5, 4, 6); G4_B(5, 6, 5, 7); G4_B(6, 7, 6, -1); G4_B(7, -1, 7, -1);
  } else if constexpr (NP == 2) {
    if (part == 0) {
      G4_R(0, 1)
      if (mw0 + 64 < M) put(std::integral_constant<int, 4>{});
      G4_K(4, 5); G4_K(5, 6); G4_K(6, 7); G4_K(7, 0);
      exchange();
      G4_B(0, 1, 0, 2); G4_B(1, 2, 1, 3); G4_B(2, 3, 2, -1); G4_B(3, -1, 3, -1);
    } else {
      G4_R(4, 5)
      if (mw0 < M) put(std::integral_constant<int, 0>{});
      G4_K(0, 1); G4_K(1, 2); G4_K(2, 3); G4_K(3, 4);
      exchange();
      G4_B(4, 5, 0, 6); G4_B(5, 6, 1, 7); G4_B(6, 7, 2, -1); G4_B(7, -1, 3, -1);
    }
  } else {
    if (part == 0) {
      G4_R(0, 1)
      if (mw0 + 48 < M) put(std::integral_constant<int, 3>{});
      G4_K(3, 4); G4_K(4, 5); G4_K(5, 6); G4_K(6, 7); G4_K(7, 0);
      exchange();
      G4_B(0, 1, 0, 2); G4_B(1, 2, 1, -1); G4_B(2, -1, 2, -1);
    } else if (part == 1) {
      G4_R(3, 4)
      if (mw0 < M) put(std::integral_constant<int, 0>{});
      G4_K(0, 1); G4_K(1, 2); G4_K(2, 7); G4_K(7, 6); G4_K(6, 3);
      exchange();
      G4_B(3, 4, 0, 5); G4_B(4, 5, 1, -1); G4_B(5, -1, 2, -1);
    } else {
      G4_R(6, 7)
      if (mw0 < M) put(std::integral_constant<int, 0>{});
      G4_K(0, 1); G4_K(1, 2); G4_K(2, 3); G4_K(3, 4); G4_K(4, 5); G4_K(5, 6);
      exchange();
      G4_B(6, 7, 0, -1); G4_B(7, -1, 1, -1);
    }
  }
#undef G4_B
#undef G4_K
#undef G4_R
  if constexpr (F16) { if (bf16_out && !qkv_tile) report_f16_overflow(f16_mx, P.f16_ovf); }
  asm volatile("s_waitcnt vmcnt(0)" ::: "memory");
  G4_STAMP(5)
#endif
}


}
```

### loongx_amd/csrc/gemm8.h

```cpp
#pragma once
#include "gemm_common.h"

#ifndef LX_ACC_AGPR
#define LX_ACC_AGPR 0
#endif

namespace {

template <int MI>
__device__ __forceinline__ void lora_issue(const lx_gemm_desc& P, int n0, int mw0, int nw0, int l31, int r0, int sp0, f32x4 (&u4)[2],
                                           f32x4 (&sv)[MI][4]) {
  const int R = P.lora_r, nsplit = P.lora_nsplit;
  const int toff = R * min(n0 / max(P.lora_mod_cols, 1), P.lora_toff_max);
  const int nvalid = min(R - r0, 4);
  const bool vec = ((R | P.lora_ldt | P.lora_split_stride | toff) & 3) == 0 && ((((uintptr_t)P.lora_t) | ((uintptr_t)P.lora_up)) & 15) == 0;
  const float* up[2];
  const float* tp[MI];
#pragma unroll
  for (int j = 0; j < 2; ++j) up[j] = P.lora_up + (size_t)min(nw0 + j * 32 + l31, P.N - 1) * R + r0;
#pragma unroll
  for (int i = 0; i < MI; ++i) tp[i] = P.lora_t + (size_t)min(mw0 + i * 32 + l31, P.M - 1) * P.lora_ldt + toff + r0;
  if (vec) {
    if (sp0 == 0) {
#pragma unroll
      for (int j = 0; j < 2; ++j) u4[j] = *(const f32x4*)up[j];
    }
#pragma unroll
    for (int i = 0; i < MI; ++i)
#pragma unroll
      for (int q = 0; q < 4; ++q) sv[i][q] = *(const f32x4*)(tp[i] + (size_t)min(sp0 + q, nsplit - 1) * P.lora_split_stride);
  } else {
    auto ld4 = [&](const float* p) {
      f32x4 v = {0.f, 0.f, 0.f, 0.f};
#pragma unroll
      for (int e = 0; e < 4; ++e)
        if (e < nvalid) v[e] = p[e];
      return v;
    };
    if (sp0 == 0) {
#pragma unroll
      for (int j = 0; j < 2; ++j) u4[j] = ld4(up[j]);
    }
#pragma unroll
    for (int i = 0; i < MI; ++i)
#pragma unroll
      for (int q = 0; q < 4; ++q) sv[i][q] = ld4(tp[i] + (size_t)min(sp0 + q, nsplit - 1) * P.lora_split_stride);
  }
}

template <int MI>
__device__ __forceinline__ void lora_sum(const lx_gemm_desc& P, int sp0, const f32x4 (&sv)[MI][4], f32x4 (&t4)[MI]) {
  const int nsplit = P.lora_nsplit;
#pragma unroll
  for (int q = 0; q < 4; ++q)
#pragma unroll
    for (int i = 0; i < MI; ++i) {
      if (sp0 + q == 0) t4[i] = sv[i][q];
      else if (sp0 + q < nsplit) {
#pragma unroll
        for (int e = 0; e < 4; ++e) t4[i][e] += sv[i][q][e];
      }
    }
}

template <int MI>
__device__ __forceinline__ void lora_apply(const f32x4 (&u4)[2], const f32x4 (&t4)[MI], int lhi, f32x16 (&acc)[2][MI]) {
  bf16x8 wf[2], xf[MI];
#pragma unroll
  for (int j = 0; j < 2; ++j) {
    u32x4 w;
#pragma unroll
    for (int e = 0; e < 2; ++e) {
      const uint16_t h0 = f32_to_bf16(u4[j][2 * e]), h1 = f32_to_bf16(u4[j][2 * e + 1]);
      w[e] = (uint32_t)h0 | ((uint32_t)h1 << 16);
      w[2 + e] = pack_bf16x2(u4[j][2 * e] - bf16_to_f32(h0), u4[j][2 * e + 1] - bf16_to_f32(h1));
    }
    wf[j] = __builtin_bit_cast(bf16x8, w);
  }
#pragma unroll
  for (int i = 0; i < MI; ++i) {
    const f32x4 t = t4[i];
    u32x2 h;
    if (lhi == 0) {
      h[0] = pack_bf16x2(t[0], t[1]);
      h[1] = pack_bf16x2(t[2], t[3]);
    } else {
      float lo[4];
#pragma unroll
      for (int e = 0; e < 4; ++e) lo[e] = t[e] - bf16_to_f32(f32_to_bf16(t[e]));
      h[0] = pack_bf16x2(lo[0], lo[1]);
      h[1] = pack_bf16x2(lo[2], lo[3]);
    }
    u32x4 x = {h[0], h[1], h[0], h[1]};
    xf[i] = __builtin_bit_cast(bf16x8, x);
  }
#pragma unroll
  for (int j = 0; j < 2; ++j)
#pragma unroll
    for (int i = 0; i < MI; ++i)
      acc[j][i] = __builtin_amdgcn_mfma_f32_32x32x16_bf16(wf[j], xf[i], acc[j][i], 0, 0, 0);
}

__device__ __forceinline__ bool lora_in_prologue(const lx_gemm_desc& P) { return P.lora_t != nullptr && P.lora_r <= 4 && P.lora_nsplit <= 4; }


template <int BM, int MI>
__device__ __forceinline__ void gemm_epilogue_qkv(const lx_gemm_desc& P, f32x16 (&acc)[2][MI], char* smem, int m0, int n0, int m_base,
                                                  int wave, int wm, int wn, int lane, int l31, int lhi) {
  const int M = P.M, D = P.qkv_d, L = P.rows_per_batch;
  const int kind = n0 / D;
  const int mw0 = m0 + wm * (BM / 2), nw0 = n0 + wn * 64;
  constexpr int EP_LD = 68;
  float* patch = (float*)smem + wave * (32 * EP_LD);
  float* ssq = (float*)smem + 8 * (32 * EP_LD);
  if (P.bias) {
#pragma unroll
    for (int j = 0; j < 2; ++j)
#pragma unroll
      for (int rq = 0; rq < 4; ++rq) {
        const f32x4 b = *(const f32x4*)(P.bias + nw0 + j * 32 + rq * 8 + 4 * lhi);
#pragma unroll
        for (int i = 0; i < MI; ++i)
#pragma unroll
          for (int c = 0; c < 4; ++c) acc[j][i][rq * 4 + c] += b[c];
      }
  }
  __syncthreads();
  auto to_patch = [&](int i) {
#pragma unroll
    for (int j = 0; j < 2; ++j)
#pragma unroll
      for (int rq = 0; rq < 4; ++rq) {
        f32x4 v = {acc[j][i][rq * 4], acc[j][i][rq * 4 + 1], acc[j][i][rq * 4 + 2], acc[j][i][rq * 4 + 3]};
        *(f32x4*)(patch + l31 * EP_LD + j * 32 + rq * 8 + 4 * lhi) = v;
      }
    __builtin_amdgcn_wave_barrier();
  };
  const bool f8 = P.qkv_q8 != nullptr;
  if (kind == 1 && f8) {
    const int h = (nw0 - D) >> 7, d0 = (nw0 - D) & 127, H = D >> 7;
    const float vs = P.qkv_v_scale;
#pragma unroll
    for (int i = 0; i < MI; ++i) {
      const int mb = mw0 + i * 32;
      if (mb >= M) continue;
      to_patch(i);
      const int gm = m_base + mb, b = gm / L, p0 = gm - b * L;
      uint8_t* vtb = (uint8_t*)P.qkv_vt8 + ((size_t)(b * H + h) * 128 + d0 + lane) * P.qkv_vt_ld + P.qkv_vt_pos0 + (p0 & ~63) + ((p0 >> 5) & 1) * 16;
#pragma unroll
      for (int g = 0; g < 2; ++g) {
        float e[16];
#pragma unroll
        for (int pp = 0; pp < 16; ++pp) e[pp] = patch[(8 * (pp >> 2) + 4 * g + (pp & 3)) * EP_LD + lane] * vs;
        u32x4 o;
#pragma unroll
        for (int q = 0; q < 4; ++q) o[q] = pack_fp8x4(e[4 * q], e[4 * q + 1], e[4 * q + 2], e[4 * q + 3]);
        *(u32x4*)(vtb + g * 32) = o;
      }
      __builtin_amdgcn_wave_barrier();
    }
    return;
  }
  if (kind == 1) {
    const int h = (nw0 - D) >> 7, d0 = (nw0 - D) & 127, H = D >> 7;
    const int dl = lane >> 2, g = lane & 3;
#pragma unroll
    for (int i = 0; i < MI; ++i) {
      const int mb = mw0 + i * 32;
      if (mb >= M) continue;
      to_patch(i);
      const int gm = m_base + mb, b = gm / L, p0 = gm - b * L;
      uint16_t* vtb = (uint16_t*)P.qkv_vt + ((size_t)(b * H + h) * 128 + d0) * P.qkv_vt_ld + P.qkv_vt_pos0 + p0 + g * 8;
#pragma unroll
      for (int it = 0; it < 4; ++it) {
        const int d = it * 16 + dl;
        float e[8];
#pragma unroll
        for (int k = 0; k < 8; ++k) e[k] = patch[lx_vt_interleave(g * 8 + k) * EP_LD + d];
        u32x4 o = {pack_bf16x2(e[0], e[1]), pack_bf16x2(e[2], e[3]), pack_bf16x2(e[4], e[5]), pack_bf16x2(e[6], e[7])};
        *(u32x4*)(vtb + (size_t)d * P.qkv_vt_ld) = o;
      }
      __builtin_amdgcn_wave_barrier();
    }
    return;
  }
#pragma unroll
  for (int i = 0; i < MI; ++i) {
    float ss = 0.f;
#pragma unroll
    for (int j = 0; j < 2; ++j)
#pragma unroll
      for (int r = 0; r < 16; ++r) ss = __builtin_fmaf(acc[j][i][r], acc[j][i][r], ss);
    ss += __shfl_xor(ss, 32, 64);
    if (lhi == 0) ssq[wave * (BM / 2) + i * 32 + l31] = ss;
  }
  const float* __restrict__ nw = kind == 2 ? P.qkv_norm_q : P.qkv_norm_k;
  const int c8 = (lane & 7) * 8;
  const int hd = (nw0 & 127) + c8;
  f32x4 w0 = *(const f32x4*)(nw + hd), w1 = *(const f32x4*)(nw + hd + 4);
  asm volatile("s_waitcnt vmcnt(0)" : "+v"(w0), "+v"(w1)::"memory");
  __syncthreads();
  const int ncol = nw0 + c8;
  uint16_t* const out = (kind == 0 && P.qkv_k) ? (uint16_t*)P.qkv_k : (uint16_t*)P.C;
  const int out_ld = (kind == 0 && P.qkv_k) ? P.qkv_k_ld : P.ldc;
  uint8_t* const out8 = f8 ? (kind == 0 ? (uint8_t*)P.qkv_k8 : (uint8_t*)P.qkv_q8) + (ncol - kind * D) : nullptr;
  const float sc8 = kind == 0 ? P.qkv_k_scale : P.qkv_q_scale;
  const float* own = ssq + wave * (BM / 2);
  const float* oth = ssq + (wave ^ 1) * (BM / 2);
  f32x4 cs[2][4][2];
  auto rope_rows = [&](int i, f32x4 (&c)[4][2]) {
    const int gm = m_base + mw0 + i * 32, b = gm / L, p0 = gm - b * L;
#pragma unroll
    for (int t = 0; t < 4; ++t) {
      const float* rp = P.qkv_rope + (size_t)(p0 + t * 8 + (lane >> 3)) * 128 + hd;
      asm volatile("global_load_dwordx4 %0, %2, off\n\tglobal_load_dwordx4 %1, %2, off offset:16" : "=&v"(c[t][0]), "=&v"(c[t][1]) : "v"(rp) : "memory");
    }
  };
  rope_rows(0, cs[0]);
#pragma unroll
  for (int i = 0; i < MI; ++i) {
    const int mb = mw0 + i * 32;
    if (mb >= M) break;
    f32x4 (&cur)[4][2] = cs[i & 1];
    to_patch(i);
    if (i == 0)
      asm volatile("s_waitcnt vmcnt(0)" : "+v"(cur[0][0]), "+v"(cur[0][1]), "+v"(cur[1][0]), "+v"(cur[1][1]), "+v"(cur[2][0]), "+v"(cur[2][1]), "+v"(cur[3][0]), "+v"(cur[3][1])::"memory");
    else
      asm volatile("s_waitcnt vmcnt(4)" : "+v"(cur[0][0]), "+v"(cur[0][1]), "+v"(cur[1][0]), "+v"(cur[1][1]), "+v"(cur[2][0]), "+v"(cur[2][1]), "+v"(cur[3][0]), "+v"(cur[3][1])::"memory");
    if (i + 1 < MI) rope_rows(i + 1, cs[(i + 1) & 1]);
#pragma unroll
    for (int t = 0; t < 4; ++t) {
      const int row = t * 8 + (lane >> 3), m = mb + row;
      const f32x4 v0 = *(const f32x4*)(patch + row * EP_LD + c8);
      const f32x4 v1 = *(const f32x4*)(patch + row * EP_LD + c8 + 4);
      const float r = rsqrtf((own[i * 32 + row] + oth[i * 32 + row]) * (1.0f / 128.0f) + 1e-6f);
      float x[8], y[8];
#pragma unroll
      for (int c = 0; c < 4; ++c) { x[c] = v0[c] * r * w0[c]; x[4 + c] = v1[c] * r * w1[c]; }
#pragma unroll
      for (int q = 0; q < 4; ++q) {
        const float co = q < 2 ? cur[t][0][2 * q] : cur[t][1][2 * q - 4], si = q < 2 ? cur[t][0][2 * q + 1] : cur[t][1][2 * q - 3];
        y[2 * q] = x[2 * q] * co - x[2 * q + 1] * si;
        y[2 * q + 1] = x[2 * q + 1] * co + x[2 * q] * si;
      }
      if (f8) {
        u32x2 o8 = {pack_fp8x4(y[0] * sc8, y[1] * sc8, y[2] * sc8, y[3] * sc8), pack_fp8x4(y[4] * sc8, y[5] * sc8, y[6] * sc8, y[7] * sc8)};
        *(u32x2*)(out8 + (size_t)m * P.qkv_ld8) = o8;
      } else {
        u32x4 o = {pack_bf16x2(y[0], y[1]), pack_bf16x2(y[2], y[3]), pack_bf16x2(y[4], y[5]), pack_bf16x2(y[6], y[7])};
        *(u32x4*)(out + (size_t)m * out_ld + ncol) = o;
      }
    }
    __builtin_amdgcn_wave_barrier();
  }
}

template <int BM, int MI, bool SPLIT = false, bool FP8 = false, bool F16 = false>
__device__ __forceinline__ void gemm_epilogue(const lx_gemm_desc& P, f32x16 (&acc)[2][MI], char* smem, int m0, int n0, int m_base,
                                              int wave, int wm, int wn, int lane, int l31, int lhi, bool lora_done, int i_begin = 0, int i_end = MI) {
  const int M = P.M, N = P.N;
  const int epi = P.epilogue & 0xff;
  const bool do_gelu = (P.epilogue & LX_EPI_GELU) != 0;
  const int mw0 = m0 + wm * (BM / 2);
  const int nw0 = n0 + wn * 64;

  if (P.lora_t != nullptr && !lora_done) {
    const int R = P.lora_r, nsplit = P.lora_nsplit;
    for (int r0 = 0; r0 < R; r0 += 4) {
      f32x4 u4[2], t4[MI];
      for (int sp0 = 0; sp0 < nsplit; sp0 += 4) {
        f32x4 sv[MI][4];
        lora_issue<MI>(P, n0, mw0, nw0, l31, r0, sp0, u4, sv);
        lora_sum<MI>(P, sp0, sv, t4);
      }
      lora_apply<MI>(u4, t4, lhi, acc);
    }
  }

  static_assert(!(F16 && (SPLIT || FP8)), "fp16 operands exclude the split-bf16 and e4m3 modes");
  if constexpr (!SPLIT && !FP8) {
    if ((P.epilogue & LX_EPI_QKV) && n0 < 3 * P.qkv_d) {
      gemm_epilogue_qkv<BM, MI>(P, acc, smem, m0, n0, m_base, wave, wm, wn, lane, l31, lhi);
      return;
    }
  }

  __syncthreads();
  constexpr int EP_LD = 68;
  float* patch = (float*)smem + wave * (32 * EP_LD);
  const bool bf16_out = epi == LX_EPI_STORE_BF16 || (FP8 && epi == LX_EPI_STORE_FP8);
  const int c8 = (lane & 7) * 8, c4 = (lane & 15) * 4;
  const int ncol = nw0 + (bf16_out ? c8 : c4);
  const bool col_ok = ncol < N;
  f32x4 bias0 = {0.f, 0.f, 0.f, 0.f}, bias1 = {0.f, 0.f, 0.f, 0.f};
  if (P.bias && col_ok) {
    bias0 = *(const f32x4*)(P.bias + ncol);
    if (bf16_out) bias1 = *(const f32x4*)(P.bias + ncol + 4);
  }
  f32x4 cs0 = {1.f, 1.f, 1.f, 1.f}, cs1 = {1.f, 1.f, 1.f, 1.f};
  if constexpr (FP8) {
    if (P.col_scale && col_ok) {
      cs0 = *(const f32x4*)(P.col_scale + ncol);
      if (bf16_out) cs1 = *(const f32x4*)(P.col_scale + ncol + 4);
    }
  }
  asm volatile("s_waitcnt vmcnt(0)" : "+v"(bias0), "+v"(bias1), "+v"(cs0), "+v"(cs1)::"memory");
  const bool gelu0 = do_gelu && ncol >= P.gelu_col_start;
  auto to_patch = [&](int i) {
#pragma unroll
    for (int j = 0; j < 2; ++j)
#pragma unroll
      for (int rq = 0; rq < 4; ++rq) {
        f32x4 v = {acc[j][i][rq * 4], acc[j][i][rq * 4 + 1], acc[j][i][rq * 4 + 2], acc[j][i][rq * 4 + 3]};
        *(f32x4*)(patch + l31 * EP_LD + j * 32 + rq * 8 + 4 * lhi) = v;
      }
    __builtin_amdgcn_wave_barrier();
  };
  if (bf16_out) {
    float f16_mx = 0.f;
#pragma unroll
    for (int i = 0; i < MI; ++i) {
      if (i < i_begin || i >= i_end) continue;
      const int mb = mw0 + i * 32;
      to_patch(i);
#pragma unroll
      for (int t = 0; t < 4; ++t) {
        const int row = t * 8 + (lane >> 3), m = mb + row;
        f32x4 v0 = *(const f32x4*)(patch + row * EP_LD + c8);
        f32x4 v1 = *(const f32x4*)(patch + row * EP_LD + c8 + 4);
        if (m < M && col_ok) {
          if constexpr (FP8) {
#pragma unroll
            for (int c = 0; c < 4; ++c) { v0[c] *= cs0[c]; v1[c] *= cs1[c]; }
          }
#pragma unroll
          for (int c = 0; c < 4; ++c) { v0[c] += bias0[c]; v1[c] += bias1[c]; }
          if (gelu0) { v0 = gelu_tanh4(v0); v1 = gelu_tanh4(v1); }
          if constexpr (FP8) {
            if (epi == LX_EPI_STORE_FP8) {
              const float os = P.out_scale;
              *(u32x2*)((uint8_t*)P.C + (size_t)m * P.ldc + ncol) = u32x2{pack_fp8x4(v0[0] * os, v0[1] * os, v0[2] * os, v0[3] * os),
                                                                          pack_fp8x4(v1[0] * os, v1[1] * os, v1[2] * os, v1[3] * os)};
              continue;
            }
          }
          u32x4 o = {pack_op16x2<F16>(v0[0], v0[1], f16_mx), pack_op16x2<F16>(v0[2], v0[3], f16_mx), pack_op16x2<F16>(v1[0], v1[1], f16_mx),
                     pack_op16x2<F16>(v1[2], v1[3], f16_mx)};
          *(u32x4*)((uint16_t*)P.C + (size_t)m * P.ldc + ncol) = o;
          if constexpr (SPLIT) {
            if (P.epilogue & LX_EPI_SPLIT_BF16) {
              float r[8];
#pragma unroll
              for (int c = 0; c < 4; ++c) {
                r[c] = v0[c] - bf16_to_f32(f32_to_bf16(v0[c]));
                r[4 + c] = v1[c] - bf16_to_f32(f32_to_bf16(v1[c]));
              }
              u32x4 ol = {pack_bf16x2(r[0], r[1]), pack_bf16x2(r[2], r[3]), pack_bf16x2(r[4], r[5]), pack_bf16x2(r[6], r[7])};
              *(u32x4*)((uint16_t*)P.C + (size_t)m * P.ldc + ncol + P.c_lo_off) = ol;
            }
          }
        }
      }
      __builtin_amdgcn_wave_barrier();
    }
    if constexpr (F16) report_f16_overflow(f16_mx, P.f16_ovf);
  } else if (epi == LX_EPI_RESID_F32) {
#pragma unroll
    for (int i = 0; i < MI; ++i) {
      if (i < i_begin || i >= i_end) continue;
      const int mb = mw0 + i * 32;
      f32x4 res[8], gat[8];
      const int rpb = P.rows_per_batch;
      const int b_first = (m_base + mb) / rpb, rem_first = (m_base + mb) - b_first * rpb;
#pragma unroll
      for (int t = 0; t < 8; ++t) {
        const int rr = t * 4 + (lane >> 4), m = mb + rr;
        if (m < M && col_ok) {
          res[t] = *(const f32x4*)((const float*)P.C + (size_t)m * P.ldc + ncol);
          const int b = rpb >= 32 ? b_first + (rem_first + rr >= rpb ? 1 : 0) : (m_base + m) / rpb;
          if (P.gate) gat[t] = *(const f32x4*)(P.gate + (size_t)b * P.gate_ld + ncol);
        }
      }
      to_patch(i);
      asm volatile("s_waitcnt vmcnt(0)" ::: "memory");
#pragma unroll
      for (int t = 0; t < 8; ++t) asm volatile("" : "+v"(res[t]), "+v"(gat[t]));
#pragma unroll
      for (int t = 0; t < 8; ++t) {
        const int row = t * 4 + (lane >> 4), m = mb + row;
        f32x4 v = *(const f32x4*)(patch + row * EP_LD + c4);
        if (m < M && col_ok) {
          if constexpr (FP8) {
#pragma unroll
            for (int c = 0; c < 4; ++c) v[c] *= cs0[c];
          }
#pragma unroll
          for (int c = 0; c < 4; ++c) v[c] += bias0[c];
          if (gelu0) v = gelu_tanh4(v);
          f32x4 o = res[t];
          if (P.gate) {
#pragma unroll
            for (int c = 0; c < 4; ++c) o[c] = __builtin_fmaf(gat[t][c], v[c], o[c]);
          } else {
#pragma unroll
            for (int c = 0; c < 4; ++c) o[c] += v[c];
          }
          *(f32x4*)((float*)P.C + (size_t)m * P.ldc + ncol) = o;
        }
      }
      __builtin_amdgcn_wave_barrier();
    }
  } else {
#pragma unroll
    for (int i = 0; i < MI; ++i) {
      if (i < i_begin || i >= i_end) continue;
      const int mb = mw0 + i * 32;
      to_patch(i);
#pragma unroll
      for (int t = 0; t < 8; ++t) {
        const int row = t * 4 + (lane >> 4), m = mb + row;
        f32x4 v = *(const f32x4*)(patch + row * EP_LD + c4);
        if (m < M && col_ok) {
          if constexpr (FP8) {
#pragma unroll
            for (int c = 0; c < 4; ++c) v[c] *= cs0[c];
          }
#pragma unroll
          for (int c = 0; c < 4; ++c) v[c] += bias0[c];
          if (gelu0) v = gelu_tanh4(v);
          *(f32x4*)((float*)P.C + (size_t)m * P.ldc + ncol) = v;
        }
      }
      __builtin_amdgcn_wave_barrier();
    }
  }
}

template <int BM>
constexpr int gemm_lds_bytes() { return BM == 128 ? 3 * (128 * BK * 2) + 3 * (BN * BK * 2) : 2 * (256 * BK * 2) + 2 * (BN * BK * 2); }

template <int BM, bool SPLIT = false, bool F16 = false, class F>
__device__ __forceinline__ void gemm_mainloop(const lx_gemm_desc& P, const int m0, const int n0, const int tn, const int kt0, const int kt1,
                                              char* smem, f32x16 (&acc)[2][BM / 64], const int tid, F&& after_issue) {
  constexpr int MI = BM / 64;
  constexpr int A_BYTES = BM * BK * 2;
  constexpr int W_BYTES = BN * BK * 2;
  constexpr int NSA = BM == 128 ? 3 : 2;
  constexpr int NSW = BM == 128 ? 3 : 2;
  constexpr int W_BASE = NSA * A_BYTES;
  constexpr int WAIT_STEADY = BM == 128 ? MI + 4 : (NSW == 3 ? 4 : 0);
  static_assert(W_BASE + NSW * W_BYTES <= 160 * 1024, "LDS budget");
  static_assert(W_BASE + NSW * W_BYTES >= 8 * 32 * 68 * 4, "epilogue patch must fit");
  static_assert(W_BASE + NSW * W_BYTES == gemm_lds_bytes<BM>(), "gemm_lds_bytes out of sync with the ring layout");

  const int lane = tid & 63;
  const int wave = __builtin_amdgcn_readfirstlane(tid >> 6);
  const int wm = wave >> 2, wn = wave & 3;
  const int l31 = lane & 31, lhi = lane >> 5;
  const int M = P.M, N = P.N, K = P.K;
  const bool w_tiled = (P.epilogue & LX_W_TILED) != 0;

  uint32_t aoff[MI], woff[4];
  {
    const int rsub = lane >> 3, pslot = lane & 7;
#pragma unroll
    for (int j = 0; j < MI; ++j) {
      const int row = (j * 8 + wave) * 8 + rsub;
      const int lslot = pslot ^ ((row >> 1) & 7);
      aoff[j] = (uint32_t)((min(m0 + row, M - 1) - m0) * P.lda + lslot * 8) * 2u;
    }
#pragma unroll
    for (int j = 0; j < 4; ++j) {
      if (w_tiled) {
        woff[j] = (uint32_t)((j * 8 + wave) * 512 + lane * 8) * 2u;
      } else {
        const int row = (j * 8 + wave) * 8 + rsub;
        const int lslot = pslot ^ ((row >> 1) & 7);
        woff[j] = (uint32_t)((min(n0 + row, N - 1) - n0) * P.ldw + lslot * 8) * 2u;
      }
    }
  }
  const int nk1 = K / BK;
  const int kw_tiles = SPLIT && P.k_segs == 3 ? 2 * nk1 : nk1;
  const __bf16* a_org = (const __bf16*)P.A + (size_t)m0 * P.lda;
  const __bf16* w_org = w_tiled ? (const __bf16*)P.W + ((size_t)tn * kw_tiles) * (BN * BK) : (const __bf16*)P.W + (size_t)n0 * P.ldw;
  const lx_rsrc_t rs_a = lx_make_rsrc(a_org), rs_w = lx_make_rsrc(w_org);
  const int w_kstride_b = (w_tiled ? BN * BK : BK) * 2;
  auto a_soff = [&](int t) -> int {
    if constexpr (!SPLIT) return t * (BK * 2);
    else {
      const int seg = t >= 2 * nk1 ? 2 : (t >= nk1 ? 1 : 0);
      return (t - seg * nk1) * (BK * 2) + (seg == 1 ? P.a_lo_off * 2 : 0);
    }
  };
  auto w_soff = [&](int t) -> int {
    if constexpr (!SPLIT) return t * w_kstride_b;
    else {
      const int seg = t >= 2 * nk1 ? 2 : (t >= nk1 ? 1 : 0);
      return (t - seg * nk1 + (seg == 2 ? nk1 : 0)) * w_kstride_b;
    }
  };
  auto stage_a = [&](int kt, int slot) {
    char* base = smem + slot * A_BYTES;
    const int so = a_soff(kt0 + kt);
#pragma unroll
    for (int j = 0; j < MI; ++j)
      lx_buf_to_lds(rs_a, (lptr_t)(base + (j * 8 + wave) * 1024), aoff[j], so);
  };
  auto stage_w = [&](int kt, int slot) {
    char* base = smem + W_BASE + slot * W_BYTES;
    const int so = w_soff(kt0 + kt);
#pragma unroll
    for (int j = 0; j < 4; ++j)
      lx_buf_to_lds(rs_w, (lptr_t)(base + (j * 8 + wave) * 1024), woff[j], so);
  };

  const int sw = (l31 >> 1) & 7;
  int slot_off[4];
#pragma unroll
  for (int ks = 0; ks < 4; ++ks) slot_off[ks] = ((ks * 2 + lhi) ^ sw) * 16;
  const int a_row_off = (wm * (BM / 2) + l31) * 128;
  const int w_row_off = (wn * 64 + l31) * 128;

  auto load_frags = [&](int sa, int sw_, int ks, bf16x8 (&wf)[2], bf16x8 (&xf)[MI]) {
    const char* pa = smem + sa * A_BYTES + a_row_off + slot_off[ks];
    const char* pw = smem + W_BASE + sw_ * W_BYTES + w_row_off + slot_off[ks];
#pragma unroll
    for (int j = 0; j < 2; ++j) wf[j] = *(const bf16x8*)(pw + j * 32 * 128);
#pragma unroll
    for (int i = 0; i < MI; ++i) xf[i] = *(const bf16x8*)(pa + i * 32 * 128);
  };
  auto mma_j = [&](int j, const bf16x8 (&wf)[2], const bf16x8 (&xf)[MI]) {
#pragma unroll
    for (int i = 0; i < MI; ++i) {
      if constexpr (F16) acc[j][i] = __builtin_amdgcn_mfma_f32_32x32x16_f16(__builtin_bit_cast(f16x8, wf[j]), __builtin_bit_cast(f16x8, xf[i]), acc[j][i], 0, 0, 0);
      else if (LX_ACC_AGPR) asm volatile("v_mfma_f32_32x32x16_bf16 %0, %1, %2, %0" : "+a"(acc[j][i]) : "v"(wf[j]), "v"(xf[i]));
      else acc[j][i] = __builtin_amdgcn_mfma_f32_32x32x16_bf16(wf[j], xf[i], acc[j][i], 0, 0, 0);
    }
  };
  const int nkt = kt1 - kt0;
  bf16x8 wfA[2], xfA[MI], wfB[2], xfB[MI];
  {
    stage_a(0, 0);
    stage_w(0, 0);
    if (nkt > 1) { stage_a(1, 1); stage_w(1, 1); }
    if (nkt > 2) { if constexpr (NSA > 2) stage_a(2, 2); if constexpr (NSW > 2) stage_w(2, 2); }
    after_issue();
    if (nkt > 2 && NSW > 2) {
      asm volatile("s_waitcnt vmcnt(12)" ::: "memory");
    } else {
      asm volatile("s_waitcnt vmcnt(0)" ::: "memory");
    }
    static_assert((BM == 128 && 2 * (MI + 4) == 12) || (BM == 256 && MI + 4 + 4 == 12), "prologue wait count");
  }
  __syncthreads();
  load_frags(0, 0, 0, wfA, xfA);
#define LX_STEP(CUR_W, CUR_X, NEXT_STMT)            \
  __builtin_amdgcn_s_setprio(1);                    \
  mma_j(0, CUR_W, CUR_X);                           \
  __builtin_amdgcn_s_setprio(0);                    \
  __builtin_amdgcn_sched_barrier(0);                \
  NEXT_STMT;                                        \
  __builtin_amdgcn_sched_barrier(0);                \
  __builtin_amdgcn_s_setprio(1);                    \
  mma_j(1, CUR_W, CUR_X);                           \
  __builtin_amdgcn_s_setprio(0);                    \
  __builtin_amdgcn_sched_barrier(0);
  int ca = 0, cw = 0;
  for (int kt = 0; kt < nkt; ++kt) {
    const int na = ca + 1 == NSA ? 0 : ca + 1;
    const int nw = cw + 1 == NSW ? 0 : cw + 1;
    LX_STEP(wfA, xfA, load_frags(ca, cw, 1, wfB, xfB))
    LX_STEP(wfB, xfB, load_frags(ca, cw, 2, wfA, xfA))
    LX_STEP(wfA, xfA, load_frags(ca, cw, 3, wfB, xfB))
    if (kt + 2 < nkt && WAIT_STEADY > 0) {
      if constexpr (WAIT_STEADY == 4) asm volatile("s_waitcnt vmcnt(4) lgkmcnt(0)" ::: "memory");
      else asm volatile("s_waitcnt vmcnt(6) lgkmcnt(0)" ::: "memory");
    } else {
      asm volatile("s_waitcnt vmcnt(0) lgkmcnt(0)" ::: "memory");
    }
    __builtin_amdgcn_s_barrier();
    __builtin_amdgcn_sched_barrier(0);
    if (wm == 0) {
      if (kt + NSA < nkt) stage_a(kt + NSA, ca);
      if (kt + NSW < nkt) stage_w(kt + NSW, cw);
    }
    __builtin_amdgcn_sched_barrier(0);
    LX_STEP(wfB, xfB, if (kt + 1 < nkt) load_frags(na, nw, 0, wfA, xfA))
    if (wm == 1) {
      if (kt + NSA < nkt) stage_a(kt + NSA, ca);
      if (kt + NSW < nkt) stage_w(kt + NSW, cw);
    }
    __builtin_amdgcn_sched_barrier(0);
    ca = na;
    cw = nw;
  }
#undef LX_STEP
  if (LX_ACC_AGPR) asm volatile("s_nop 15\n s_nop 7" ::: "memory");
}

template <int MI>
__device__ __forceinline__ void acc_clear(f32x16 (&acc)[2][MI]) {
#pragma unroll
  for (int j = 0; j < 2; ++j)
#pragma unroll
    for (int i = 0; i < MI; ++i)
#pragma unroll
      for (int r = 0; r < 16; ++r) acc[j][i][r] = 0.f;
}

template <int BM, bool SPLIT = false, bool F16 = false>
__device__ __forceinline__ void gemm_tile(const GemmArgs& args, const int pid, char* smem) {
  constexpr int MI = BM / 64;
  const int total = args.tile_start[MAX_SUB];
  int lid;
  {
    const int q = total >> 3, r = total & 7;
    const int xcd = pid & 7, inx = pid >> 3;
    lid = (xcd < r ? xcd * (q + 1) : r * (q + 1) + (xcd - r) * q) + inx;
  }
  const int g = tile_group(args, lid);
  const lx_gemm_desc P = args.p[g];
  int tm, tn;
  tile_coords<BM>(P, lid - args.tile_start[g], tm, tn);
  const int tid = threadIdx.x, lane = tid & 63;
  const int wave = __builtin_amdgcn_readfirstlane(tid >> 6);
  f32x16 acc[2][MI];
  acc_clear<MI>(acc);
  const int wm = wave >> 2, wn = wave & 3, l31 = lane & 31, lhi = lane >> 5;
  const int m0 = tm * BM, n0 = tn * BN;
  const bool lora_early = lora_in_prologue(P);
  f32x4 u4[2], sv[MI][4];
  if (lora_early) lora_issue<MI>(P, n0, m0 + wm * (BM / 2), n0 + wn * 64, l31, 0, 0, u4, sv);
  const int nkt = SPLIT ? (P.K / BK) * max(P.k_segs, 1) : P.K / BK;
  gemm_mainloop<BM, SPLIT, F16>(P, m0, n0, tn, 0, nkt, smem, acc, tid, [&]() {
    if (lora_early) {
      f32x4 t4[MI];
      lora_sum<MI>(P, 0, sv, t4);
      lora_apply<MI>(u4, t4, lhi, acc);
    }
  });
  gemm_epilogue<BM, MI, SPLIT, false, F16>(P, acc, smem, m0, n0, args.m_base[g], wave, wm, wn, lane, l31, lhi, lora_early);
}

template <int BM, bool F16 = false>
__global__ __launch_bounds__(NTHREADS) void lx_gemm_kernel(const GemmArgs args) {
  __shared__ __attribute__((aligned(1024))) char smem[gemm_lds_bytes<BM>()];
  gemm_tile<BM, false, F16>(args, blockIdx.x, smem);
}

template <int BM>
__global__ __launch_bounds__(NTHREADS) void lx_gemm_split_kernel(const GemmArgs args) {
  __shared__ __attribute__((aligned(1024))) char smem[gemm_lds_bytes<BM>()];
  gemm_tile<BM, true>(args, blockIdx.x, smem);
}

typedef int i32x8 __attribute__((ext_vector_type(8)));

template <int BM, class F>
__device__ __forceinline__ void gemm_mainloop_fp8(const lx_gemm_desc& P, const int m0, const int n0, const int tn, const int kt0, const int kt1,
                                                  char* smem, f32x16 (&acc)[2][BM / 64], const int tid, F&& after_issue) {
  constexpr int MI = BM / 64;
  constexpr int KB = 128;
  constexpr int A_BYTES = BM * KB;
  constexpr int W_BYTES = BN * KB;
  constexpr int NSA = BM == 128 ? 3 : 2;
  constexpr int NSW = BM == 128 ? 3 : 2;
  constexpr int W_BASE = NSA * A_BYTES;
  constexpr int WAIT_STEADY = BM == 128 ? MI + 4 : 0;
  static_assert(W_BASE + NSW * W_BYTES == gemm_lds_bytes<BM>(), "fp8 rings must have the bf16 rings' geometry");
  const int lane = tid & 63;
  const int wave = __builtin_amdgcn_readfirstlane(tid >> 6);
  const int wm = wave >> 2, wn = wave & 3;
  const int l31 = lane & 31, lhi = lane >> 5;
  const int M = P.M, N = P.N, K = P.K;
  const bool w_tiled = (P.epilogue & LX_W_TILED) != 0;
  uint32_t aoff[MI], woff[4];
  {
    const int rsub = lane >> 3, pslot = lane & 7;
#pragma unroll
    for (int j = 0; j < MI; ++j) {
      const int row = (j * 8 + wave) * 8 + rsub;
      const int lslot = pslot ^ ((row >> 1) & 7);
      aoff[j] = (uint32_t)((min(m0 + row, M - 1) - m0) * P.lda + lslot * 16);
    }
#pragma unroll
    for (int j = 0; j < 4; ++j) {
      if (w_tiled) {
        woff[j] = (uint32_t)((j * 8 + wave) * 1024 + lane * 16);
      } else {
        const int row = (j * 8 + wave) * 8 + rsub;
        const int lslot = pslot ^ ((row >> 1) & 7);
        woff[j] = (uint32_t)((min(n0 + row, N - 1) - n0) * P.ldw + lslot * 16);
      }
    }
  }
  const uint8_t* a_org = (const uint8_t*)P.A + (size_t)m0 * P.lda;
  const uint8_t* w_org = w_tiled ? (const uint8_t*)P.W + ((size_t)tn * (K / KB)) * (BN * KB) : (const uint8_t*)P.W + (size_t)n0 * P.ldw;
  const lx_rsrc_t rs_a = lx_make_rsrc(a_org), rs_w = lx_make_rsrc(w_org);
  const int w_kstride_b = w_tiled ? BN * KB : KB;
  auto stage_a = [&](int kt, int slot) {
    char* base = smem + slot * A_BYTES;
#pragma unroll
    for (int j = 0; j < MI; ++j) lx_buf_to_lds(rs_a, (lptr_t)(base + (j * 8 + wave) * 1024), aoff[j], (kt0 + kt) * KB);
  };
  auto stage_w = [&](int kt, int slot) {
    char* base = smem + W_BASE + slot * W_BYTES;
#pragma unroll
    for (int j = 0; j < 4; ++j) lx_buf_to_lds(rs_w, (lptr_t)(base + (j * 8 + wave) * 1024), woff[j], (kt0 + kt) * w_kstride_b);
  };
  const int sw = (l31 >> 1) & 7;
  int slot_off[2][2];
#pragma unroll
  for (int ks = 0; ks < 2; ++ks)
#pragma unroll
    for (int h = 0; h < 2; ++h) slot_off[ks][h] = ((ks * 4 + lhi * 2 + h) ^ sw) * 16;
  const int a_row_off = (wm * (BM / 2) + l31) * 128;
  const int w_row_off = (wn * 64 + l31) * 128;
  auto frag = [&](const char* p, int ks) {
    const u32x4 lo = *(const u32x4*)(p + slot_off[ks][0]), hi = *(const u32x4*)(p + slot_off[ks][1]);
    return i32x8{(int)lo[0], (int)lo[1], (int)lo[2], (int)lo[3], (int)hi[0], (int)hi[1], (int)hi[2], (int)hi[3]};
  };
  auto load_frags = [&](int sa, int sw_, int ks, i32x8 (&wf)[2], i32x8 (&xf)[MI]) {
    const char* pa = smem + sa * A_BYTES + a_row_off;
    const char* pw = smem + W_BASE + sw_ * W_BYTES + w_row_off;
#pragma unroll
    for (int j = 0; j < 2; ++j) wf[j] = frag(pw + j * 32 * 128, ks);
#pragma unroll
    for (int i = 0; i < MI; ++i) xf[i] = frag(pa + i * 32 * 128, ks);
  };
  auto mma_j = [&](int j, const i32x8 (&wf)[2], const i32x8 (&xf)[MI]) {
#pragma unroll
    for (int i = 0; i < MI; ++i) acc[j][i] = __builtin_amdgcn_mfma_scale_f32_32x32x64_f8f6f4(wf[j], xf[i], acc[j][i], 0, 0, 0, 0, 0, 0);
  };
  const int nkt = kt1 - kt0;
  i32x8 wfA[2], xfA[MI], wfB[2], xfB[MI];
  {
    stage_a(0, 0);
    stage_w(0, 0);
    if (nkt > 1) { stage_a(1, 1); stage_w(1, 1); }
    if (nkt > 2) { if constexpr (NSA > 2) stage_a(2, 2); if constexpr (NSW > 2) stage_w(2, 2); }
    after_issue();
    if (nkt > 2 && NSW > 2) {
      asm volatile("s_waitcnt vmcnt(12)" ::: "memory");
    } else {
      asm volatile("s_waitcnt vmcnt(0)" ::: "memory");
    }
  }
  __syncthreads();
  load_frags(0, 0, 0, wfA, xfA);
#define LX_STEP8(CUR_W, CUR_X, NEXT_STMT)           \
  __builtin_amdgcn_s_setprio(1);                    \
  mma_j(0, CUR_W, CUR_X);                           \
  __builtin_amdgcn_s_setprio(0);                    \
  __builtin_amdgcn_sched_barrier(0);                \
  NEXT_STMT;                                        \
  __builtin_amdgcn_sched_barrier(0);                \
  __builtin_amdgcn_s_setprio(1);                    \
  mma_j(1, CUR_W, CUR_X);                           \
  __builtin_amdgcn_s_setprio(0);                    \
  __builtin_amdgcn_sched_barrier(0);
  int ca = 0, cw = 0;
  for (int kt = 0; kt < nkt; ++kt) {
    const int na = ca + 1 == NSA ? 0 : ca + 1;
    const int nw = cw + 1 == NSW ? 0 : cw + 1;
    LX_STEP8(wfA, xfA, load_frags(ca, cw, 1, wfB, xfB))
    if (kt + 2 < nkt && WAIT_STEADY > 0) {
      asm volatile("s_waitcnt vmcnt(6) lgkmcnt(0)" ::: "memory");
    } else {
      asm volatile("s_waitcnt vmcnt(0) lgkmcnt(0)" ::: "memory");
    }
    __builtin_amdgcn_s_barrier();
    __builtin_amdgcn_sched_barrier(0);
    if (wm == 0) {
      if (kt + NSA < nkt) stage_a(kt + NSA, ca);
      if (kt + NSW < nkt) stage_w(kt + NSW, cw);
    }
    __builtin_amdgcn_sched_barrier(0);
    LX_STEP8(wfB, xfB, if (kt + 1 < nkt) load_frags(na, nw, 0, wfA, xfA))
    if (wm == 1) {
      if (kt + NSA < nkt) stage_a(kt + NSA, ca);
      if (kt + NSW < nkt) stage_w(kt + NSW, cw);
    }
    __builtin_amdgcn_sched_barrier(0);
    ca = na;
    cw = nw;
  }
#undef LX_STEP8
}

template <int BM>
__global__ __launch_bounds__(NTHREADS) void lx_gemm_fp8_kernel(const GemmArgs args) {
  __shared__ __attribute__((aligned(1024))) char smem[gemm_lds_bytes<BM>()];
  constexpr int MI = BM / 64;
  const int pid = blockIdx.x;
  const int total = args.tile_start[MAX_SUB];
  int lid;
  {
    const int q = total >> 3, r = total & 7;
    const int xcd = pid & 7, inx = pid >> 3;
    lid = (xcd < r ? xcd * (q + 1) : r * (q + 1) + (xcd - r) * q) + inx;
  }
  const int g = tile_group(args, lid);
  const lx_gemm_desc P = args.p[g];
  int tm, tn;
  tile_coords<BM>(P, lid - args.tile_start[g], tm, tn);
  const int tid = threadIdx.x, lane = tid & 63;
  const int wave = __builtin_amdgcn_readfirstlane(tid >> 6);
  f32x16 acc[2][MI];
  acc_clear<MI>(acc);
  const int wm = wave >> 2, wn = wave & 3, l31 = lane & 31, lhi = lane >> 5;
  const int m0 = tm * BM, n0 = tn * BN;
  const bool lora_early = lora_in_prologue(P);
  f32x4 u4[2], sv[MI][4];
  if (lora_early) lora_issue<MI>(P, n0, m0 + wm * (BM / 2), n0 + wn * 64, l31, 0, 0, u4, sv);
  gemm_mainloop_fp8<BM>(P, m0, n0, tn, 0, P.K / 128, smem, acc, tid, [&]() {
    if (lora_early) {
      f32x4 t4[MI];
      lora_sum<MI>(P, 0, sv, t4);
      if (P.col_scale) {
#pragma unroll
        for (int j = 0; j < 2; ++j) {
          const float inv = 1.0f / P.col_scale[min(n0 + wn * 64 + j * 32 + l31, P.N - 1)];
#pragma unroll
          for (int e = 0; e < 4; ++e) u4[j][e] *= inv;
        }
      }
      lora_apply<MI>(u4, t4, lhi, acc);
    }
  });
  gemm_epilogue<BM, MI, false, true>(P, acc, smem, m0, n0, args.m_base[g], wave, wm, wn, lane, l31, lhi, lora_early);
}

template <bool F16 = false>
__global__ __launch_bounds__(NTHREADS) void lx_gemm_mixed_kernel(const GemmArgs big, const GemmArgs tail, const int n_big_pad) {
  __shared__ __attribute__((aligned(1024))) char smem[gemm_lds_bytes<128>() > gemm_lds_bytes<256>() ? gemm_lds_bytes<128>() : gemm_lds_bytes<256>()];
  const int bid = blockIdx.x;
  if (bid < big.tile_start[MAX_SUB]) gemm_tile<256, false, F16>(big, bid, smem);
  else if (bid >= n_big_pad) gemm_tile<128, false, F16>(tail, bid - n_big_pad, smem);
}


}
```

### loongx_amd/csrc/gemm_common.h

```cpp
#pragma once
#include "common.h"
#include <type_traits>

constexpr int MAX_SUB = 2 * LX_GEMM_MAX_GROUP;

struct GemmArgs {
  lx_gemm_desc p[MAX_SUB];
  int tile_start[MAX_SUB + 1];
  int m_base[MAX_SUB];
  int n;
};
static_assert(2 * sizeof(GemmArgs) + 16 <= 4096, "lx_gemm_mixed_kernel takes two plans by value: the kernarg segment is 4 KiB");

namespace {

constexpr int BN = 256;
constexpr int BK = 64;
constexpr int NTHREADS = 512;
#ifndef LX_GROUP_M
#define LX_GROUP_M 4
#endif
constexpr int GROUP_M = LX_GROUP_M;

typedef const __attribute__((address_space(1))) void* gptr_t;
typedef __attribute__((address_space(3))) void* lptr_t;

constexpr int PAIR_AUX_SC1 = 16;

__device__ __forceinline__ int tile_group(const GemmArgs& args, const int lid) {
  int g = 0;
#pragma unroll
  for (int i = 1; i < MAX_SUB; ++i)
    if (lid >= args.tile_start[i]) g = i;
  return g;
}

template <int BM>
__device__ __forceinline__ void tile_coords(const lx_gemm_desc& P, const int local, int& tm, int& tn) {
  const int tiles_m = (P.M + BM - 1) / BM;
  const int tiles_n = (P.N + BN - 1) / BN;
  const int gs = GROUP_M * tiles_n;
  const int gi = local / gs, in_g = local - gi * gs;
  const int first_m = gi * GROUP_M;
  const int gm = min(tiles_m - first_m, GROUP_M);
  tm = first_m + in_g % gm;
  tn = in_g / gm;
}

constexpr int G4_THREADS = 256;
constexpr int SK_SLOT_FLOATS = 256 * 256;

}

enum { LX_GV_BF16 = 0, LX_GV_F16 = 1, LX_GV_SPLIT = 2, LX_GV_FP8 = 3 };

void lx_gemm8_launch_bf16(int bm, const GemmArgs& a, hipStream_t s);
void lx_gemm8_launch_f16(int bm, const GemmArgs& a, hipStream_t s);
void lx_gemm8_launch_split(int bm, const GemmArgs& a, hipStream_t s);
void lx_gemm8_launch_fp8(int bm, const GemmArgs& a, hipStream_t s);
void lx_gemm8_mixed_launch_bf16(const GemmArgs& big, const GemmArgs& tail, int n_big_pad, hipStream_t s);
void lx_gemm8_mixed_launch_f16(const GemmArgs& big, const GemmArgs& tail, int n_big_pad, hipStream_t s);
void lx_gemm4_launch_bf16(const GemmArgs& a, unsigned grid, int sk_full, int sk_parts, float* slots, int* flags, int* err, hipStream_t s, int np = 2);
void lx_gemm4_launch_f16(const GemmArgs& a, unsigned grid, int sk_full, int sk_parts, float* slots, int* flags, int* err, hipStream_t s, int np = 2);
void lx_gemm4_launch_split(const GemmArgs& a, unsigned grid, int sk_full, int sk_parts, float* slots, int* flags, int* err, hipStream_t s);
```

### loongx_amd/csrc/gemm_f16.hip

```cpp
#include "gemm8.h"

void lx_gemm8_launch_f16(int bm, const GemmArgs& a, hipStream_t s) {
  const int t = a.tile_start[a.n];
  if (bm == 256) hipLaunchKernelGGL((lx_gemm_kernel<256, true>), dim3(t), dim3(NTHREADS), 0, s, a);
  else hipLaunchKernelGGL((lx_gemm_kernel<128, true>), dim3(t), dim3(NTHREADS), 0, s, a);
}
void lx_gemm8_mixed_launch_f16(const GemmArgs& big, const GemmArgs& tail, int n_big_pad, hipStream_t s) {
  hipLaunchKernelGGL(lx_gemm_mixed_kernel<true>, dim3(n_big_pad + tail.tile_start[tail.n]), dim3(NTHREADS), 0, s, big, tail, n_big_pad);
}
```

### loongx_amd/csrc/gemm_modes.hip

```cpp
#include "gemm8.h"

void lx_gemm8_launch_split(int bm, const GemmArgs& a, hipStream_t s) {
  const int t = a.tile_start[a.n];
  if (bm == 256) hipLaunchKernelGGL(lx_gemm_split_kernel<256>, dim3(t), dim3(NTHREADS), 0, s, a);
  else hipLaunchKernelGGL(lx_gemm_split_kernel<128>, dim3(t), dim3(NTHREADS), 0, s, a);
}
void lx_gemm8_launch_fp8(int bm, const GemmArgs& a, hipStream_t s) {
  const int t = a.tile_start[a.n];
  if (bm == 256) hipLaunchKernelGGL(lx_gemm_fp8_kernel<256>, dim3(t), dim3(NTHREADS), 0, s, a);
  else hipLaunchKernelGGL(lx_gemm_fp8_kernel<128>, dim3(t), dim3(NTHREADS), 0, s, a);
}
```

Measured before the change: 1.052.

## Precompute compact per-group tile descriptors and magic-number tile mapping for GEMM kernels

Moves per-subproblem tile-mapping data into a compact 64-byte descriptor block. Each kernel prologue now loads only that block and replaces integer divisions with precomputed magic multiplies. The g4 kernel issues its first two K-tile prefetches before loading the full problem descriptor and LoRA operands, so the prologue latency overlaps. It also shrinks the plan to four subproblems and adds host-side tile-map query APIs plus a tile-count range check. The costs are a new limit on problem size or count and a changed wait count in the LoRA path.

```diff
diff --git a/include/lx.h b/include/lx.h
--- a/include/lx.h
+++ b/include/lx.h
@@ -80,6 +80,9 @@
 enum { LX_GEMM_PLAN_NONE = 0, LX_GEMM_PLAN_8WAVE_256 = 1, LX_GEMM_PLAN_8WAVE_128 = 2, LX_GEMM_PLAN_MIXED = 3, LX_GEMM_PLAN_MIXED_2L = 4,
        LX_GEMM_PLAN_G4 = 5, LX_GEMM_PLAN_G4_SPLIT2 = 6, LX_GEMM_PLAN_G4_SPLIT3 = 7 };
 int lx_gemm_last_plan(void);
+int lx_gemm_tile_map(int32_t* out, int cap);
+int lx_gemm_tile_map_shapes(const int32_t* mn, int n, int bm, const int32_t* mn_tail, int n_tail, int sk_full, int np, int32_t* out, int cap);
+uint32_t lx_gemm_tile_magic(uint32_t d);
 
 int lx_lora_down(const void* X, int ldx, const void* Adown, float* T, int ldt, int M, int K, int R, int n_split,
                  int split_stride, void* stream);
diff --git a/loongx_amd/_lib.py b/loongx_amd/_lib.py
--- a/loongx_amd/_lib.py
+++ b/loongx_amd/_lib.py
@@ -85,6 +85,9 @@
     "lx_gemm_bf16_ws": (C.c_int, [C.POINTER(GemmDesc), _I, _P, _Z, _P]),
     "lx_gemm_workspace_status": (C.c_int, [_P, _P]),
     "lx_gemm_last_plan": (C.c_int, []),
+    "lx_gemm_tile_map": (C.c_int, [C.POINTER(C.c_int32), _I]),
+    "lx_gemm_tile_map_shapes": (C.c_int, [C.POINTER(C.c_int32), _I, _I, C.POINTER(C.c_int32), _I, _I, _I, C.POINTER(C.c_int32), _I]),
+    "lx_gemm_tile_magic": (C.c_uint32, [C.c_uint32]),
     "lx_lora_down": (C.c_int, [_P, _I, _P, _P, _I, _I, _I, _I, _I, _I, _P]),
     "lx_lora_down_f16": (C.c_int, [_P, _I, _P, _P, _I, _I, _I, _I, _I, _I, _P]),
     "lx_lora_down_terms": (C.c_int, [C.POINTER(C.c_void_p), C.POINTER(C.c_int), C.POINTER(C.c_void_p), _I, _P, _I, _I, _I, _I, _I, _P]),
diff --git a/loongx_amd/csrc/gemm.hip b/loongx_amd/csrc/gemm.hip
--- a/loongx_amd/csrc/gemm.hip
+++ b/loongx_amd/csrc/gemm.hip
@@ -48,8 +48,10 @@
   return q;
 }
 
+static void map_note_8wave(const GemmArgs& a, int bm);
 static int launch_plan(const GemmArgs& a, int bm, hipStream_t s, int variant = LX_GV_BF16) {
-  if (a.n == 0) return LX_OK;
+  if (a.t.n == 0) return LX_OK;
+  map_note_8wave(a, bm);
   if (variant == LX_GV_SPLIT) lx_gemm8_launch_split(bm, a, s);
   else if (variant == LX_GV_F16) lx_gemm8_launch_f16(bm, a, s);
   else if (variant == LX_GV_FP8) lx_gemm8_launch_fp8(bm, a, s);
@@ -59,20 +61,24 @@
 }
 
 void lx_gemm8_launch_bf16(int bm, const GemmArgs& a, hipStream_t s) {
-  const int t = a.tile_start[a.n];
+  const int t = a.t.tile_start[a.t.n];
   if (bm == 256) hipLaunchKernelGGL((lx_gemm_kernel<256, false>), dim3(t), dim3(NTHREADS), 0, s, a);
   else hipLaunchKernelGGL((lx_gemm_kernel<128, false>), dim3(t), dim3(NTHREADS), 0, s, a);
 }
 void lx_gemm8_mixed_launch_bf16(const GemmArgs& big, const GemmArgs& tail, int n_big_pad, hipStream_t s) {
-  hipLaunchKernelGGL(lx_gemm_mixed_kernel<false>, dim3(n_big_pad + tail.tile_start[tail.n]), dim3(NTHREADS), 0, s, big, tail, n_big_pad);
-}
-
+  hipLaunchKernelGGL(lx_gemm_mixed_kernel<false>, dim3(n_big_pad + tail.t.tile_start[tail.t.n]), dim3(NTHREADS), 0, s, big, tail, n_big_pad);
+}
+
+static void plan_init(GemmArgs& a) {
+  a = GemmArgs{};
+}
 static void plan_add(GemmArgs& a, const lx_gemm_desc& p, int m_base, int bm) {
-  a.p[a.n] = p;
-  a.m_base[a.n] = m_base;
-  a.tile_start[a.n + 1] = a.tile_start[a.n] + (int)tiles_of(p, bm);
-  ++a.n;
-  for (int i = a.n + 1; i <= MAX_SUB; ++i) a.tile_start[i] = a.tile_start[a.n];
+  lx_tile_plan& t = a.t;
+  a.p[t.n] = p;
+  t.st[t.n] = lx_tile_start_fill(p, bm, m_base, t.tile_start[t.n]);
+  t.tile_start[t.n + 1] = t.tile_start[t.n] + (int)tiles_of(p, bm);
+  ++t.n;
+  for (int i = t.n + 1; i <= PLAN_SUB; ++i) t.tile_start[i] = t.tile_start[t.n];
 }
 
 static thread_local int lx_gemm_last = LX_GEMM_PLAN_NONE;
@@ -81,6 +87,91 @@
   if (rc == LX_OK) lx_gemm_last = plan;
   return rc;
 }
+
+namespace {
+struct LastMap {
+  int kind = 0;
+  int bm = 0, n_big_pad = 0, grid = 0, sk_full = 0, np = 1;
+  lx_tile_plan a{}, b{};
+};
+thread_local LastMap lx_gemm_map;
+void map_8wave(const GemmArgs& a, int bm) {
+  LastMap& m = lx_gemm_map;
+  m.kind = 1; m.bm = bm; m.a = a.t; m.grid = a.t.tile_start[a.t.n];
+}
+void map_mixed(const GemmArgs& big, const GemmArgs& tail, int n_big_pad) {
+  LastMap& m = lx_gemm_map;
+  m.kind = 2; m.a = big.t; m.b = tail.t; m.n_big_pad = n_big_pad; m.grid = n_big_pad + tail.t.tile_start[tail.t.n];
+}
+void map_g4(const GemmArgs& a, unsigned grid, int sk_full, int np) {
+  LastMap& m = lx_gemm_map;
+  m.kind = 3; m.bm = 256; m.a = a.t; m.grid = (int)grid; m.sk_full = sk_full; m.np = np;
+}
+template <int BM>
+void map_tile(const lx_tile_plan& t, int lid, int sub0, int part, int32_t* o) {
+  lx_tile_start R;
+  const int g = lx_tile_sub(t, lid, R);
+  int tm, tn;
+  lx_tile_coords<BM>(R, lid - R.t0, tm, tn);
+  o[0] = sub0 + g; o[1] = tm; o[2] = tn; o[3] = part;
+}
+}
+
+static void map_note_8wave(const GemmArgs& a, int bm) { map_8wave(a, bm); }
+
+static int map_fill(const LastMap& m, int32_t* out, int cap) {
+  if (m.kind == 0) return 0;
+  LX_CHECK_ARG(out && cap >= m.grid, "lx_gemm_tile_map: room for %d workgroups needed (cap=%d)", m.grid, cap);
+  for (int pid = 0; pid < m.grid; ++pid) {
+    int32_t* o = out + 4 * (size_t)pid;
+    if (m.kind == 1) {
+      const int lid = lx_tile_xcd_lid(pid, m.a.tile_start[PLAN_SUB]);
+      if (m.bm == 256) map_tile<256>(m.a, lid, 0, 0, o);
+      else map_tile<128>(m.a, lid, 0, 0, o);
+    } else if (m.kind == 2) {
+      const int n_big = m.a.tile_start[PLAN_SUB];
+      if (pid < n_big) map_tile<256>(m.a, lx_tile_xcd_lid(pid, n_big), 0, 0, o);
+      else if (pid >= m.n_big_pad) map_tile<128>(m.b, lx_tile_xcd_lid(pid - m.n_big_pad, m.b.tile_start[PLAN_SUB]), PLAN_SUB, 0, o);
+      else o[0] = o[1] = o[2] = o[3] = -1;
+    } else {
+      int part;
+      const int lid = lx_tile_g4_lid(pid, m.sk_full, m.np, part);
+      map_tile<256>(m.a, lid, 0, part, o);
+    }
+  }
+  return m.grid;
+}
+
+extern "C" int lx_gemm_tile_map(int32_t* out, int cap) { return map_fill(lx_gemm_map, out, cap); }
+
+extern "C" int lx_gemm_tile_map_shapes(const int32_t* mn, int n, int bm, const int32_t* mn_tail, int n_tail, int sk_full, int np, int32_t* out, int cap) {
+  LX_CHECK_ARG(mn && n >= 1 && n <= PLAN_SUB && n_tail >= 0 && n_tail <= PLAN_SUB && (bm == 256 || bm == 128) && (n_tail == 0 || mn_tail), "lx_gemm_tile_map_shapes: bad plan");
+  GemmArgs a, b;
+  plan_init(a);
+  plan_init(b);
+  lx_gemm_desc p{};
+  for (int i = 0; i < n + n_tail; ++i) {
+    const int32_t* q = i < n ? mn + 2 * i : mn_tail + 2 * (i - n);
+    LX_CHECK_ARG(q[0] > 0 && q[1] > 0, "lx_gemm_tile_map_shapes: bad shape %d x %d", q[0], q[1]);
+    p.M = q[0]; p.N = q[1];
+    LX_CHECK_ARG(lx_tile_div_exact(tiles_of(p, 128), (p.N + BN - 1) / BN), "lx_gemm_tile_map_shapes: %d x %d has too many tiles", q[0], q[1]);
+    if (i < n) plan_add(a, p, 0, n_tail ? 256 : bm);
+    else plan_add(b, p, 0, 128);
+  }
+  LastMap m;
+  const int total = a.t.tile_start[PLAN_SUB];
+  if (n_tail) {
+    m.kind = 2; m.a = a.t; m.b = b.t; m.n_big_pad = (total + 7) & ~7; m.grid = m.n_big_pad + b.t.tile_start[PLAN_SUB];
+  } else if (sk_full >= 0) {
+    LX_CHECK_ARG(bm == 256 && sk_full <= total && (np == 2 || np == 3 || sk_full == total), "lx_gemm_tile_map_shapes: bad split (sk_full=%d of %d, np=%d)", sk_full, total, np);
+    m.kind = 3; m.bm = 256; m.a = a.t; m.sk_full = sk_full; m.np = sk_full == total ? 1 : np; m.grid = sk_full + m.np * (total - sk_full);
+  } else {
+    m.kind = 1; m.bm = bm; m.a = a.t; m.grid = total;
+  }
+  return map_fill(m, out, cap);
+}
+
+extern "C" uint32_t lx_gemm_tile_magic(uint32_t d) { return d ? lx_tile_magic(d) : 0; }
 
 extern "C" size_t lx_gemm_workspace_bytes(void) { return SK_WS_BYTES; }
 
@@ -166,6 +257,7 @@
       qkv = true;
     }
     if (p.bias) LX_CHECK_ARG(((uintptr_t)p.bias & 15) == 0, "lx_gemm_bf16[%d]: bias must be 16-byte aligned", i);
+    LX_CHECK_ARG(lx_tile_div_exact(tiles_of(p, 128), (p.N + BN - 1) / BN), "lx_gemm_bf16[%d]: too many tiles for the tile map (M=%d N=%d)", i, p.M, p.N);
     t256 += tiles_of(p, 256);
     t128 += tiles_of(p, 128);
     kmax = p.K * segs > kmax ? p.K * segs : kmax;
@@ -176,9 +268,7 @@
     const double ca = (double)((t256 + ncu - 1) / ncu) * round_us(256, kmax / 4), cb = (double)((t128 + ncu - 1) / ncu) * round_us(128, kmax / 4);
     const int bm = gemm_env().bm ? gemm_env().bm : (cb < ca ? 128 : 256);
     GemmArgs all;
-    all.n = 0;
-    all.tile_start[0] = 0;
-    for (int i = 1; i <= MAX_SUB; ++i) all.tile_start[i] = 0;
+    plan_init(all);
     for (int i = 0; i < n; ++i) plan_add(all, problems[i], 0, bm);
     return planned(launch_plan(all, bm, s, LX_GV_FP8), bm == 256 ? LX_GEMM_PLAN_8WAVE_256 : LX_GEMM_PLAN_8WAVE_128);
   }
@@ -220,9 +310,7 @@
     }
     if (ok && (fills || split_all || split_tail)) {
       GemmArgs all;
-      all.n = 0;
-      all.tile_start[0] = 0;
-      for (int i = 1; i <= MAX_SUB; ++i) all.tile_start[i] = 0;
+      plan_init(all);
       for (int i = 0; i < n; ++i) plan_add(all, problems[i], 0, 256);
       float* slots = nullptr;
       int *flags = nullptr, *err = nullptr;
@@ -240,6 +328,7 @@
       else if (f16) lx_gemm4_launch_f16(all, grid, sk_full, sk_parts, slots, flags, err, s, np);
       else lx_gemm4_launch_bf16(all, grid, sk_full, sk_parts, slots, flags, err, s, np);
       LX_LAUNCH_CHECK("lx_gemm_bf16");
+      map_g4(all, grid, sk_full, (split_all || split_tail) ? np : 1);
       return planned(LX_OK, !(split_all || split_tail) ? LX_GEMM_PLAN_G4 : np == 3 ? LX_GEMM_PLAN_G4_SPLIT3 : LX_GEMM_PLAN_G4_SPLIT2);
     }
   }
@@ -247,9 +336,7 @@
     const double ca = (double)((t256 + NCU - 1) / NCU) * round_us(256, kmax), cb = (double)((t128 + NCU - 1) / NCU) * round_us(128, kmax);
     const int bm = forced ? forced : (cb < ca ? 128 : 256);
     GemmArgs all;
-    all.n = 0;
-    all.tile_start[0] = 0;
-    for (int i = 1; i <= MAX_SUB; ++i) all.tile_start[i] = 0;
+    plan_init(all);
     for (int i = 0; i < n; ++i) plan_add(all, problems[i], 0, bm);
     return planned(launch_plan(all, bm, s, LX_GV_SPLIT), bm == 256 ? LX_GEMM_PLAN_8WAVE_256 : LX_GEMM_PLAN_8WAVE_128);
   }
@@ -258,9 +345,8 @@
   const double c_a = (double)((t256 + NCU - 1) / NCU) * round_us(256, kmax);
   const double c_b = (double)((t128 + NCU - 1) / NCU) * round_us(128, kmax);
   GemmArgs big, tail;
-  big.n = tail.n = 0;
-  big.tile_start[0] = tail.tile_start[0] = 0;
-  for (int i = 1; i <= MAX_SUB; ++i) big.tile_start[i] = tail.tile_start[i] = 0;
+  plan_init(big);
+  plan_init(tail);
   double c_c = 1e30;
   const long full = (t256 / NCU) * NCU;
   if (forced == 0 && full > 0 && t256 > full) {
@@ -288,11 +374,12 @@
   }
   int choice = forced == 256 ? 0 : forced == 128 ? 1 : (c_c < c_a && c_c < c_b) ? 2 : (c_b < c_a ? 1 : 0);
   if (choice == 2) {
-    if (big.n > 0 && tail.n > 0) {
-      const int n_big = big.tile_start[big.n], n_big_pad = (n_big + 7) & ~7;
+    if (big.t.n > 0 && tail.t.n > 0) {
+      const int n_big = big.t.tile_start[big.t.n], n_big_pad = (n_big + 7) & ~7;
       if (f16) lx_gemm8_mixed_launch_f16(big, tail, n_big_pad, s);
       else lx_gemm8_mixed_launch_bf16(big, tail, n_big_pad, s);
       LX_LAUNCH_CHECK("lx_gemm_bf16");
+      map_mixed(big, tail, n_big_pad);
       return planned(LX_OK, LX_GEMM_PLAN_MIXED);
     }
     const int rc = launch_plan(big, 256, s, variant);
@@ -300,9 +387,7 @@
     return planned(launch_plan(tail, 128, s, variant), LX_GEMM_PLAN_MIXED_2L);
   }
   GemmArgs all;
-  all.n = 0;
-  all.tile_start[0] = 0;
-  for (int i = 1; i <= MAX_SUB; ++i) all.tile_start[i] = 0;
+  plan_init(all);
   for (int i = 0; i < n; ++i) plan_add(all, problems[i], 0, choice == 0 ? 256 : 128);
   return planned(launch_plan(all, choice == 0 ? 256 : 128, s, variant), choice == 0 ? LX_GEMM_PLAN_8WAVE_256 : LX_GEMM_PLAN_8WAVE_128);
 }
diff --git a/loongx_amd/csrc/gemm4.h b/loongx_amd/csrc/gemm4.h
--- a/loongx_amd/csrc/gemm4.h
+++ b/loongx_amd/csrc/gemm4.h
@@ -28,32 +28,24 @@
   constexpr int BM = 256, A_BYTES = BM * BK * 2;
   const int pid = blockIdx.x;
   G4_STAMP(0)
-  const int total = args.tile_start[MAX_SUB];
-  int lid, part = 0;
-  if (pid < sk_full) {
-    const int q = sk_full >> 3, r = sk_full & 7;
-    const int xcd = pid & 7, inx = pid >> 3;
-    lid = (xcd < r ? xcd * (q + 1) : r * (q + 1) + (xcd - r) * q) + inx;
-  } else {
-    const int r = pid - sk_full;
-    lid = sk_full + r / NP;
-    part = r % NP;
-  }
-  (void)total;
+  asm volatile("" ::"s"(sk_full), "s"(sk_parts), "s"(args.t.tile_start[1]), "s"(args.t.tile_start[2]), "s"(args.t.tile_start[3]));
+  lx_tile_start st;
+  int part;
+  const int lid = lx_tile_g4_lid(pid, sk_full, NP, part);
+  const int g = lx_tile_sub(args.t, lid, st);
   const bool split_tile = pid >= sk_full && sk_parts >= 2;
-  const int g = tile_group(args, lid);
-  lx_gemm_desc P = args.p[g];
   int tm, tn;
-  tile_coords<BM>(P, lid - args.tile_start[g], tm, tn);
+  lx_tile_coords<BM>(st, lid - st.t0, tm, tn);
   const int tid = threadIdx.x, lane = tid & 63;
   const int wave = __builtin_amdgcn_readfirstlane(tid >> 6);
   const int wm = wave >> 1, wn = wave & 1, l15 = lane & 15, lq = lane >> 4;
   int m0 = tm * BM, n0 = tn * BN;
-  int M = P.M, N = P.N;
-  const int K = P.K;
-  const bool w_tiled = (P.epilogue & LX_W_TILED) != 0;
+  int M = st.M, N = st.N;
+  const int K = st.K;
+  const bool w_tiled = (st.flags & 1) != 0;
+  const int k_segs = SPLIT ? (st.flags >> 8) & 3 : 1;
   const int nk1 = K / BK;
-  const int nkt = SPLIT ? nk1 * max(P.k_segs, 1) : nk1;
+  const int nkt = SPLIT ? nk1 * max(k_segs, 1) : nk1;
   const int kt_begin = !split_tile ? 0 : NP == 2 ? (part ? nkt >> 1 : 0) : (part * nkt) / NP;
   const int kt_end = !split_tile ? nkt : NP == 2 ? (part ? nkt : nkt >> 1) : ((part + 1) * nkt) / NP;
 
@@ -64,16 +56,16 @@
     for (int j = 0; j < 8; ++j) {
       const int row = (j * 4 + wave) * 8 + rsub;
       const int lslot = pslot ^ ((row >> 1) & 7);
-      aoff[j] = (uint32_t)((min(m0 + row, M - 1) - m0) * P.lda + lslot * 8) * 2u;
-      woff[j] = w_tiled ? (uint32_t)((j * 4 + wave) * 512 + lane * 8) * 2u : (uint32_t)((min(n0 + row, N - 1) - n0) * P.ldw + lslot * 8) * 2u;
-    }
-  }
-  const __bf16* a_org = (const __bf16*)P.A + (size_t)m0 * P.lda;
-  const int kw_tiles = SPLIT && P.k_segs == 3 ? 2 * nk1 : nk1;
-  const __bf16* w_org = w_tiled ? (const __bf16*)P.W + ((size_t)tn * kw_tiles) * (BN * BK) : (const __bf16*)P.W + (size_t)n0 * P.ldw;
+      aoff[j] = (uint32_t)((min(m0 + row, M - 1) - m0) * st.lda + lslot * 8) * 2u;
+      woff[j] = w_tiled ? (uint32_t)((j * 4 + wave) * 512 + lane * 8) * 2u : (uint32_t)((min(n0 + row, N - 1) - n0) * st.ldw + lslot * 8) * 2u;
+    }
+  }
+  const __bf16* a_org = (const __bf16*)st.A + (size_t)m0 * st.lda;
+  const int kw_tiles = SPLIT && k_segs == 3 ? 2 * nk1 : nk1;
+  const __bf16* w_org = w_tiled ? (const __bf16*)st.W + ((size_t)tn * kw_tiles) * (BN * BK) : (const __bf16*)st.W + (size_t)n0 * st.ldw;
   const lx_rsrc_t rs_a = lx_make_rsrc(a_org), rs_w = lx_make_rsrc(w_org);
   const int w_kstride_b = (w_tiled ? BN * BK : BK) * 2;
-  const int a_lo_b = SPLIT ? P.a_lo_off * 2 : 0;
+  const int a_lo_b = SPLIT ? st.a_lo_off * 2 : 0;
   auto a_soff = [&](int t) -> int {
     if constexpr (!SPLIT) return t * (BK * 2);
     else {
@@ -118,6 +110,17 @@
     else asm volatile("v_mfma_f32_16x16x32_bf16 %0, %1, %2, %0" : "+a"(acc[i][j]) : "v"(wf[ks][j]), "v"(af[ks][i]));
   };
 #define G4_SB() __builtin_amdgcn_sched_barrier(0)
+  {
+    const int t1 = min(kt_begin + 1, kt_end - 1);
+    const int a0 = a_soff(kt_begin), w0 = w_soff(kt_begin), a1 = a_soff(t1), w1 = w_soff(t1);
+#pragma unroll
+    for (int p_ = 0; p_ < 16; ++p_) piece(p_, a0, w0, 0);
+#pragma unroll
+    for (int p_ = 0; p_ < 16; ++p_) piece(p_, a1, w1, 1);
+  }
+  int g_late = g;
+  asm volatile("" : "+s"(g_late)::"memory");
+  const lx_gemm_desc P = args.p[g_late];
   const bool has_lora = P.lora_t != nullptr && kt_begin == 0;
   u32x2 lu[8], lt[8][4];
   if (has_lora) {
@@ -133,15 +136,8 @@
       for (int q = 0; q < 4; ++q) lt[i][q] = *(const u32x2*)(tp + (size_t)min(q, nsplit - 1) * P.lora_split_stride);
     }
   }
-  {
-    const int t1 = min(kt_begin + 1, kt_end - 1);
-    const int a0 = a_soff(kt_begin), w0 = w_soff(kt_begin), a1 = a_soff(t1), w1 = w_soff(t1);
-#pragma unroll
-    for (int p_ = 0; p_ < 16; ++p_) piece(p_, a0, w0, 0);
-#pragma unroll
-    for (int p_ = 0; p_ < 16; ++p_) piece(p_, a1, w1, 1);
-  }
-  asm volatile("s_waitcnt vmcnt(16)" ::: "memory");
+  if (has_lora) asm volatile("s_waitcnt vmcnt(56)" ::: "memory");
+  else asm volatile("s_waitcnt vmcnt(16)" ::: "memory");
   __builtin_amdgcn_s_barrier();
   G4_SB();
   G4_STAMP(1)
@@ -290,7 +286,7 @@
   }
   asm volatile("s_waitcnt vmcnt(0)" : "+v"(bias0), "+v"(bias1)::"memory");
   const bool gelu0 = do_gelu && ncol >= P.gelu_col_start;
-  const int m_base = args.m_base[g];
+  const int m_base = st.m_base;
   static_assert(!(F16 && SPLIT), "fp16 operands exclude the split-bf16 mode");
   float f16_mx = 0.f;
   const bool qkv_tile = (P.epilogue & LX_EPI_QKV) != 0 && n0 < 3 * P.qkv_d;
diff --git a/loongx_amd/csrc/gemm8.h b/loongx_amd/csrc/gemm8.h
--- a/loongx_amd/csrc/gemm8.h
+++ b/loongx_amd/csrc/gemm8.h
@@ -612,17 +612,13 @@
 template <int BM, bool SPLIT = false, bool F16 = false>
 __device__ __forceinline__ void gemm_tile(const GemmArgs& args, const int pid, char* smem) {
   constexpr int MI = BM / 64;
-  const int total = args.tile_start[MAX_SUB];
-  int lid;
-  {
-    const int q = total >> 3, r = total & 7;
-    const int xcd = pid & 7, inx = pid >> 3;
-    lid = (xcd < r ? xcd * (q + 1) : r * (q + 1) + (xcd - r) * q) + inx;
-  }
-  const int g = tile_group(args, lid);
+  const int total = args.t.tile_start[PLAN_SUB];
+  const int lid = lx_tile_xcd_lid(pid, total);
+  lx_tile_start R;
+  const int g = lx_tile_sub(args.t, lid, R);
+  int tm, tn;
+  lx_tile_coords<BM>(R, lid - R.t0, tm, tn);
   const lx_gemm_desc P = args.p[g];
-  int tm, tn;
-  tile_coords<BM>(P, lid - args.tile_start[g], tm, tn);
   const int tid = threadIdx.x, lane = tid & 63;
   const int wave = __builtin_amdgcn_readfirstlane(tid >> 6);
   f32x16 acc[2][MI];
@@ -640,7 +636,7 @@
       lora_apply<MI>(u4, t4, lhi, acc);
     }
   });
-  gemm_epilogue<BM, MI, SPLIT, false, F16>(P, acc, smem, m0, n0, args.m_base[g], wave, wm, wn, lane, l31, lhi, lora_early);
+  gemm_epilogue<BM, MI, SPLIT, false, F16>(P, acc, smem, m0, n0, R.m_base, wave, wm, wn, lane, l31, lhi, lora_early);
 }
 
 template <int BM, bool F16 = false>
@@ -794,17 +790,13 @@
   __shared__ __attribute__((aligned(1024))) char smem[gemm_lds_bytes<BM>()];
   constexpr int MI = BM / 64;
   const int pid = blockIdx.x;
-  const int total = args.tile_start[MAX_SUB];
-  int lid;
-  {
-    const int q = total >> 3, r = total & 7;
-    const int xcd = pid & 7, inx = pid >> 3;
-    lid = (xcd < r ? xcd * (q + 1) : r * (q + 1) + (xcd - r) * q) + inx;
-  }
-  const int g = tile_group(args, lid);
+  const int total = args.t.tile_start[PLAN_SUB];
+  const int lid = lx_tile_xcd_lid(pid, total);
+  lx_tile_start R;
+  const int g = lx_tile_sub(args.t, lid, R);
+  int tm, tn;
+  lx_tile_coords<BM>(R, lid - R.t0, tm, tn);
   const lx_gemm_desc P = args.p[g];
-  int tm, tn;
-  tile_coords<BM>(P, lid - args.tile_start[g], tm, tn);
   const int tid = threadIdx.x, lane = tid & 63;
   const int wave = __builtin_amdgcn_readfirstlane(tid >> 6);
   f32x16 acc[2][MI];
@@ -829,14 +821,14 @@
       lora_apply<MI>(u4, t4, lhi, acc);
     }
   });
-  gemm_epilogue<BM, MI, false, true>(P, acc, smem, m0, n0, args.m_base[g], wave, wm, wn, lane, l31, lhi, lora_early);
+  gemm_epilogue<BM, MI, false, true>(P, acc, smem, m0, n0, R.m_base, wave, wm, wn, lane, l31, lhi, lora_early);
 }
 
 template <bool F16 = false>
 __global__ __launch_bounds__(NTHREADS) void lx_gemm_mixed_kernel(const GemmArgs big, const GemmArgs tail, const int n_big_pad) {
   __shared__ __attribute__((aligned(1024))) char smem[gemm_lds_bytes<128>() > gemm_lds_bytes<256>() ? gemm_lds_bytes<128>() : gemm_lds_bytes<256>()];
   const int bid = blockIdx.x;
-  if (bid < big.tile_start[MAX_SUB]) gemm_tile<256, false, F16>(big, bid, smem);
+  if (bid < big.t.tile_start[PLAN_SUB]) gemm_tile<256, false, F16>(big, bid, smem);
   else if (bid >= n_big_pad) gemm_tile<128, false, F16>(tail, bid - n_big_pad, smem);
 }
 
diff --git a/loongx_amd/csrc/gemm_common.h b/loongx_amd/csrc/gemm_common.h
--- a/loongx_amd/csrc/gemm_common.h
+++ b/loongx_amd/csrc/gemm_common.h
@@ -3,49 +3,102 @@
 #include <type_traits>
 
 constexpr int MAX_SUB = 2 * LX_GEMM_MAX_GROUP;
+constexpr int PLAN_SUB = LX_GEMM_MAX_GROUP;
 
-struct GemmArgs {
-  lx_gemm_desc p[MAX_SUB];
-  int tile_start[MAX_SUB + 1];
-  int m_base[MAX_SUB];
+struct lx_tile_start {
+  const void* A;
+  const void* W;
+  int32_t M, N, K;
+  int32_t lda, ldw;
+  int32_t gs;
+  uint32_t gs_mul;
+  uint32_t tail_mul;
+  int32_t a_lo_off;
+  int32_t m_base;
+  int32_t t0;
+  int32_t flags;
+};
+static_assert(sizeof(lx_tile_start) == 64, "one s_load_dwordx16");
+
+struct lx_tile_plan {
+  lx_tile_start st[PLAN_SUB];
+  int tile_start[PLAN_SUB + 1];
   int n;
 };
+struct GemmArgs {
+  lx_tile_plan t;
+  lx_gemm_desc p[PLAN_SUB];
+};
 static_assert(2 * sizeof(GemmArgs) + 16 <= 4096, "lx_gemm_mixed_kernel takes two plans by value: the kernarg segment is 4 KiB");
+
+#ifndef LX_GROUP_M
+#define LX_GROUP_M 4
+#endif
+constexpr int LX_TILE_GROUP_M = LX_GROUP_M;
+__host__ __device__ inline bool lx_tile_div_exact(long long tiles, long long tiles_n) { return tiles * LX_TILE_GROUP_M * tiles_n < (1ll << 31); }
+__host__ __device__ inline uint32_t lx_tile_magic(uint32_t d) { return (uint32_t)(((1ull << 31) + d - 1) / d); }
+__host__ __device__ inline int lx_tile_div(int x, uint32_t mul) { return (int)(((uint64_t)((uint32_t)x << 1) * mul) >> 32); }
+
+__host__ __device__ inline int lx_tile_xcd_lid(int pid, int total) {
+  const int q = total >> 3, r = total & 7;
+  const int xcd = pid & 7, inx = pid >> 3;
+  return (xcd < r ? xcd * (q + 1) : r * (q + 1) + (xcd - r) * q) + inx;
+}
+__host__ __device__ inline int lx_tile_sub(const lx_tile_plan& args, int lid, lx_tile_start& R) {
+  int g = 0;
+#pragma unroll
+  for (int i = 1; i < PLAN_SUB; ++i) g += lid >= args.tile_start[i] ? 1 : 0;
+  R = args.st[g];
+#if defined(__HIP_DEVICE_COMPILE__)
+  asm volatile("" ::"s"(R.A), "s"(R.W), "s"(R.M), "s"(R.N), "s"(R.K), "s"(R.lda), "s"(R.ldw), "s"(R.gs), "s"(R.gs_mul), "s"(R.tail_mul), "s"(R.a_lo_off),
+               "s"(R.m_base), "s"(R.t0), "s"(R.flags));
+#endif
+  return g;
+}
+template <int BM>
+__host__ __device__ inline void lx_tile_coords(const lx_tile_start& R, int local, int& tm, int& tn) {
+  const int tiles_m = (R.M + BM - 1) / BM;
+  const int gi = lx_tile_div(local, R.gs_mul), in_g = local - gi * R.gs;
+  const int first_m = gi * LX_TILE_GROUP_M;
+  const bool whole = tiles_m - first_m >= LX_TILE_GROUP_M;
+  const int gm = whole ? LX_TILE_GROUP_M : tiles_m - first_m;
+  tn = whole ? in_g / LX_TILE_GROUP_M : lx_tile_div(in_g, R.tail_mul);
+  tm = first_m + in_g - tn * gm;
+}
+__host__ __device__ inline int lx_tile_g4_lid(int pid, int sk_full, int np, int& part) {
+  part = 0;
+  if (pid < sk_full) return lx_tile_xcd_lid(pid, sk_full);
+  const int r = pid - sk_full;
+  part = r % np;
+  return sk_full + r / np;
+}
+inline lx_tile_start lx_tile_start_fill(const lx_gemm_desc& p, int bm, int m_base, int t0) {
+  lx_tile_start r;
+  const int tiles_m = (p.M + bm - 1) / bm, tiles_n = (p.N + 255) / 256, tail_h = tiles_m % LX_TILE_GROUP_M ? tiles_m % LX_TILE_GROUP_M : LX_TILE_GROUP_M;
+  r.A = p.A; r.W = p.W;
+  r.M = p.M; r.N = p.N; r.K = p.K;
+  r.lda = p.lda; r.ldw = p.ldw;
+  r.gs = LX_TILE_GROUP_M * tiles_n;
+  r.gs_mul = lx_tile_magic((uint32_t)r.gs);
+  r.tail_mul = lx_tile_magic((uint32_t)tail_h);
+  r.a_lo_off = p.a_lo_off;
+  r.m_base = m_base;
+  r.t0 = t0;
+  r.flags = ((p.epilogue & LX_W_TILED) ? 1 : 0) | ((p.k_segs & 3) << 8);
+  return r;
+}
 
 namespace {
 
 constexpr int BN = 256;
 constexpr int BK = 64;
 constexpr int NTHREADS = 512;
-#ifndef LX_GROUP_M
-#define LX_GROUP_M 4
-#endif
 constexpr int GROUP_M = LX_GROUP_M;
 
 typedef const __attribute__((address_space(1))) void* gptr_t;
 typedef __attribute__((address_space(3))) void* lptr_t;
 
 constexpr int PAIR_AUX_SC1 = 16;
-
-__device__ __forceinline__ int tile_group(const GemmArgs& args, const int lid) {
-  int g = 0;
-#pragma unroll
-  for (int i = 1; i < MAX_SUB; ++i)
-    if (lid >= args.tile_start[i]) g = i;
-  return g;
-}
-
-template <int BM>
-__device__ __forceinline__ void tile_coords(const lx_gemm_desc& P, const int local, int& tm, int& tn) {
-  const int tiles_m = (P.M + BM - 1) / BM;
-  const int tiles_n = (P.N + BN - 1) / BN;
-  const int gs = GROUP_M * tiles_n;
-  const int gi = local / gs, in_g = local - gi * gs;
-  const int first_m = gi * GROUP_M;
-  const int gm = min(tiles_m - first_m, GROUP_M);
-  tm = first_m + in_g % gm;
-  tn = in_g / gm;
-}
 
 constexpr int G4_THREADS = 256;
 constexpr int SK_SLOT_FLOATS = 256 * 256;
diff --git a/loongx_amd/csrc/gemm_f16.hip b/loongx_amd/csrc/gemm_f16.hip
--- a/loongx_amd/csrc/gemm_f16.hip
+++ b/loongx_amd/csrc/gemm_f16.hip
@@ -1,10 +1,10 @@
 #include "gemm8.h"
 
 void lx_gemm8_launch_f16(int bm, const GemmArgs& a, hipStream_t s) {
-  const int t = a.tile_start[a.n];
+  const int t = a.t.tile_start[a.t.n];
   if (bm == 256) hipLaunchKernelGGL((lx_gemm_kernel<256, true>), dim3(t), dim3(NTHREADS), 0, s, a);
   else hipLaunchKernelGGL((lx_gemm_kernel<128, true>), dim3(t), dim3(NTHREADS), 0, s, a);
 }
 void lx_gemm8_mixed_launch_f16(const GemmArgs& big, const GemmArgs& tail, int n_big_pad, hipStream_t s) {
-  hipLaunchKernelGGL(lx_gemm_mixed_kernel<true>, dim3(n_big_pad + tail.tile_start[tail.n]), dim3(NTHREADS), 0, s, big, tail, n_big_pad);
+  hipLaunchKernelGGL(lx_gemm_mixed_kernel<true>, dim3(n_big_pad + tail.t.tile_start[tail.t.n]), dim3(NTHREADS), 0, s, big, tail, n_big_pad);
 }
diff --git a/loongx_amd/csrc/gemm_modes.hip b/loongx_amd/csrc/gemm_modes.hip
--- a/loongx_amd/csrc/gemm_modes.hip
+++ b/loongx_amd/csrc/gemm_modes.hip
@@ -1,12 +1,12 @@
 #include "gemm8.h"
 
 void lx_gemm8_launch_split(int bm, const GemmArgs& a, hipStream_t s) {
-  const int t = a.tile_start[a.n];
+  const int t = a.t.tile_start[a.t.n];
   if (bm == 256) hipLaunchKernelGGL(lx_gemm_split_kernel<256>, dim3(t), dim3(NTHREADS), 0, s, a);
   else hipLaunchKernelGGL(lx_gemm_split_kernel<128>, dim3(t), dim3(NTHREADS), 0, s, a);
 }
 void lx_gemm8_launch_fp8(int bm, const GemmArgs& a, hipStream_t s) {
-  const int t = a.tile_start[a.n];
+  const int t = a.t.tile_start[a.t.n];
   if (bm == 256) hipLaunchKernelGGL(lx_gemm_fp8_kernel<256>, dim3(t), dim3(NTHREADS), 0, s, a);
   else hipLaunchKernelGGL(lx_gemm_fp8_kernel<128>, dim3(t), dim3(NTHREADS), 0, s, a);
 }
```

Measured after the change: 1.055 (median of 6 runs). Within noise of the previous version (+0.3%).
